# scottschroeder/shirley-raytracing-rs

Hardware: AMD Instinct MI355X
Metric: Msamples/sec (whole node) on book-1 random_scene 1200x800 @ 500spp; 1/2/4/8 GPU (higher is better)
Workload: dtype f64

## Files before the change

### include/shirley_rt.h

```cpp
#ifndef SHIRLEY_RT_H
#define SHIRLEY_RT_H

#include <stddef.h>
#include <stdint.h>

#ifdef __cplusplus
extern "C" {
#endif

#define RT_ABI_VERSION 11

typedef enum rt_status {
  RT_OK = 0,
  RT_E_INVALID = 1,
  RT_E_HIP = 2,
  RT_E_OOM = 3,
  RT_E_UNSUPPORTED = 4,
  RT_E_RCCL = 5
} rt_status;

enum { RT_GEOM_SPHERE = 0, RT_GEOM_RECT_XY = 1, RT_GEOM_RECT_YZ = 2, RT_GEOM_RECT_XZ = 3, RT_GEOM_RECT_BOX = 4,
       RT_GEOM_MOVING_SPHERE = 5 };
enum { RT_MAT_METAL = 0, RT_MAT_DIELECTRIC = 1, RT_MAT_LAMBERTIAN = 2, RT_MAT_DIFFUSE_LIGHT = 3, RT_MAT_FAIRY_LIGHT = 4,
       RT_MAT_ISOTROPIC = 5 };
// ... 67 lines not shown
  int32_t n_perlin;
  const rt_perlin_table* perlin;
  int32_t n_images;
  const rt_image* images;
} rt_scene_desc;

typedef struct rt_camera {
  int32_t image_width;
  int32_t image_height;
  double height;
  double width;
  double focal_length;
  int32_t has_lens;
  double lens_radius;
  double origin[3];
  double w[3], u[3], v[3];
  double focus_length;
  double time0, time1;
} rt_camera;

typedef struct rt_render_params {
  int32_t samples;
  int32_t max_depth;
  uint64_t seed;
  int32_t tile_rank;
  int32_t tile_world;
  int32_t sample_chunk;
  int32_t engine;
  int32_t sample_begin;
  int32_t sample_count;
  int32_t partition;
  int32_t scratch_mb;
} rt_render_params;

enum {
  RT_PARTITION_AUTO = 0,
  RT_PARTITION_TILES = 1,
  RT_PARTITION_SAMPLES = 2
};

typedef struct rt_scene_stats {
  int32_t n_objects;
  int32_t n_nodes;
  int32_t n_leaves;
  int32_t depth;
  int64_t device_bytes;
  int32_t n_nodes4;
  int32_t wide_block;
  double origin_limit;
  int32_t hop_pass;
  int32_t hop_kind;
} rt_scene_stats;

typedef struct rt_counters {
  uint64_t samples;
  uint64_t segments;
  uint64_t node_visits;
  uint64_t prim_tests;
  double kernel_ms;
  double reduce_ms;
  int32_t engine;
  int32_t iterations;
  uint64_t slots;
  double extend_ms;
  double shade_ms;
  double texture_ms;
  int32_t sample_chunk;
  int32_t n_chunks;
  int32_t passes;
  int32_t trace_launches;
  uint64_t scratch_bytes;
} rt_counters;

typedef struct rt_ctx rt_ctx;

const char* rt_version(void);
int rt_device_count(int32_t* out);
int rt_create(int32_t device, rt_ctx** out);
int rt_destroy(rt_ctx* ctx);
const char* rt_last_error(const rt_ctx* ctx);

int rt_scene_upload(rt_ctx* ctx, const rt_scene_desc* scene, int32_t bvh_builder);
int rt_scene_stats_get(rt_ctx* ctx, rt_scene_stats* out);
int rt_scene_digest(rt_ctx* ctx, uint64_t* out);
int rt_scene_digest_host(const rt_scene_desc* scene, int32_t bvh_builder, uint64_t* out);

int rt_render(rt_ctx* ctx, const rt_camera* cam, const rt_render_params* params, double* accum_host);

int rt_render_scanlines(rt_ctx* ctx, const rt_camera* cam, const rt_render_params* params,
                        int32_t line_begin, int32_t line_end, double* rows_host);

int rt_tile_layout(const rt_camera* cam, int32_t tile_world, int32_t* n_tiles_total, int32_t* max_tiles_per_rank);
int rt_render_device(rt_ctx* ctx, const rt_camera* cam, const rt_render_params* params, double* accum_dev,
                     void* stream);
int rt_render_tiles_device(rt_ctx* ctx, const rt_camera* cam, const rt_render_params* params,
                           double* packed_dev, void* stream);
int rt_unpack_tiles_device(rt_ctx* ctx, const rt_camera* cam, int32_t tile_world, const double* gathered_dev,
                           double* accum_dev, void* stream);
int rt_synchronize(rt_ctx* ctx);

typedef struct rt_hit {
  int32_t object;
  int32_t front_face;
  double t;
  double point[3];
  double normal[3];
  double u, v;
} rt_hit;
int rt_scene_hit(rt_ctx* ctx, const double* rays, int32_t n, double t_min, double t_max, rt_hit* out);

enum { RT_TRAVERSAL_BINARY = 0, RT_TRAVERSAL_RENDER = 1 };
int rt_scene_hit_ex(rt_ctx* ctx, const double* rays, int32_t n, double t_min, double t_max, int32_t traversal,
                    rt_hit* out);

typedef struct rt_probe {
  int32_t object;
  int32_t front_face;
  int32_t scattered;
  int32_t emits;
  uint32_t draw;
  int32_t pad;
  double t, point[3], normal[3];
  double emitted[3];
  double attenuation[3];
  double origin[3], direction[3];
} rt_probe;
int rt_probe_segment(rt_ctx* ctx, const double* rays, int32_t n, uint64_t seed, uint32_t sample, uint32_t draw,
                     rt_probe* out);

#define RT_COMM_ID_BYTES 128
typedef struct rt_comm rt_comm;
int rt_comm_unique_id(uint8_t id[RT_COMM_ID_BYTES]);
int rt_comm_init_rank(rt_ctx* ctx, const uint8_t id[RT_COMM_ID_BYTES], int32_t world, int32_t rank, rt_comm** out);
int rt_comm_destroy(rt_comm* comm);
int rt_render_sharded(rt_ctx* ctx, rt_comm* comm, const rt_camera* cam, const rt_render_params* params,
                      double* accum_dev, void* stream);
int rt_render_multi(rt_ctx* const* ctxs, int32_t n, const rt_camera* cam, const rt_render_params* params,
                    double* accum_host);

int rt_counters_get(rt_ctx* ctx, rt_counters* out);

typedef struct rt_bvh_node {
  double box[6];
  int32_t leaf;
  int32_t lhs, rhs;
  int32_t pad;
} rt_bvh_node;
int rt_bvh_build_host(const rt_scene_desc* scene, int32_t bvh_builder, int32_t* n_nodes, rt_bvh_node* nodes,
                      int32_t* root);

int rt_tonemap(const double* accum, int32_t width, int32_t height, int32_t samples, uint8_t* rgb8);
int rt_tonemap_device(rt_ctx* ctx, const double* accum_dev, int32_t width, int32_t height, int32_t samples,
                      uint8_t* rgb8_dev, void* stream);

typedef struct rt_adaptive_params {
  int32_t min_samples;
  int32_t step;
  double  threshold;
  double  noise_floor;
} rt_adaptive_params;

typedef struct rt_adaptive_report {
  int32_t  steps, tiles, tiles_converged, pad;
  uint64_t samples, segments;
  double   kernel_ms, fold_ms;
} rt_adaptive_report;
// ... 93 lines not shown
```

### shirley-raytracing-rs_amd/csrc/rt/rt_api.cpp

```cpp
#include <algorithm>
#include <cmath>
#include <cstdlib>
#include <cstring>
#include <limits>
#include <string>
#include <vector>

#include "adaptive.h"
#include "plan.h"
#include "rt_ctx.h"

using namespace rt;

namespace rt {

int ensure(rt_ctx* c, DevBuf& b, size_t bytes) {
  if (b.bytes >= bytes && b.p) return RT_OK;
  if (c) HIP_TRY(c, hipSetDevice(c->device));
  if (b.p) {
    (void)hipFree(b.p);
    b.p = nullptr;
    b.bytes = 0;
  }
  if (bytes == 0) return RT_OK;
// ... 288 lines not shown
  kp.work.tiles_x = L.tiles_x;
  kp.work.tiles_y = L.tiles_y;
  kp.work.ty0 = ty0;
  kp.work.tile_rank = p->tile_rank;
  kp.work.tile_world = p->tile_world;
  kp.work.n_tiles_rank = L.n_tiles_rank;
  kp.work.chunk = chunk;
  kp.work.max_depth = p->max_depth;
  kp.work.seed = p->seed;
  kp.work.div_tiles_x = make_udiv((uint32_t)L.tiles_x);
  kp.work.tile_list = step ? step->list_dev : nullptr;
  kp.partial = static_cast<double*>(c->partial.p);
  kp.counters = static_cast<DCounters*>(c->counters.p);

  st = ensure(c, c->kcam, (size_t)passes * sizeof(KBlock));
  if (st) return st;
  kp.scene.shutter = &static_cast<KBlock*>(c->kcam.p)->scene.time0;
  c->host_blocks.assign(passes, KBlock{});
  const uint64_t nseg = (uint64_t)std::max(1, c->cu_count * std::max(1, c->blocks_per_cu));
  {
    const size_t bytes = std::max<size_t>(64, (size_t)nseg * sizeof(uint32_t));
    st = ensure(c, c->unit_counter, bytes);
    if (st) return st;
    kp.unit_counter = static_cast<unsigned long long*>(c->unit_counter.p);
  }
  if ((int)c->pass_ev.size() < 2 * passes) {
    const size_t have = c->pass_ev.size();
    c->pass_ev.resize(2 * passes, nullptr);
    for (size_t i = have; i < c->pass_ev.size(); ++i) HIP_TRY(c, hipEventCreate(&c->pass_ev[i]));
  }
  HIP_TRY(c, hipMemsetAsync(c->counters.p, 0, kCounterSlots * sizeof(DCounters), s));
  c->last_engine = engine;
  c->host_samples = 0;
  c->last_chunk = chunk;
  c->last_n_chunks = n_chunks;
  c->last_passes = 0;
  c->last_scratch = partial_bytes;
  c->last_iters = 0;
  c->last_slots = 0;
  c->last_timing = 0;
  for (double& x : c->lap_ms) x = 0.0;
  HIP_TRY(c, hipEventRecord(c->ev[0], s));
  const bool trace = n_pix > 0 && count > 0 && p->max_depth > 0;
  if (step && (!trace || chunk != step->batch)) return fail(c, RT_E_INVALID, "bad adaptive step");
  if (!trace) {
    uint64_t inside = 0;
    for (long long lt = 0; lt < L.n_tiles_rank; ++lt) {
      const long long gt = lt * p->tile_world + p->tile_rank;
      const int tx = (int)(gt % L.tiles_x), ty = ty0 + (int)(gt / L.tiles_x);
      const int w = std::min(kTile, cam->image_width - tx * kTile), h = std::min(kTile, cam->image_height - ty * kTile);
      if (w > 0 && h > 0) inside += (uint64_t)w * (uint64_t)h;
    }
    c->host_samples = inside * (uint64_t)count;
    HIP_TRY(c, hipEventRecord(c->ev[1], s));
    if (n_pix > 0)
      HIP_TRY(c, launch_reduce(kp.partial, 0, L.n_tiles_rank, L.tiles_x, ty0, p->tile_rank, p->tile_world,
                               cam->image_width, row0, row1, packed, 0, out_dev, s));
    HIP_TRY(c, hipEventRecord(c->ev[2], s));
    c->have_timing = true;
    return RT_OK;
  }
  for (int k = 0; k < passes; ++k) {
    const int c0 = k * per_pass, c1 = std::min(n_chunks, c0 + per_pass);
    DWork& w = kp.work;
    w.sample_base = R.begin + c0 * chunk;
    w.samples = (int)std::min<long long>(R.end, (long long)R.begin + (long long)c1 * chunk);
    w.n_chunks = c1 - c0;
    w.n_units = (uint64_t)n_pix * (uint64_t)w.n_chunks;
    w.div_unit_tile = make_udiv((uint32_t)w.n_chunks * (uint32_t)kTilePixels);
    const uint64_t per = (w.n_units + nseg - 1) / nseg;
    w.n_segs = plan.segments ? (uint32_t)nseg : 0u;
    w.seg_len = (uint32_t)std::max<uint64_t>(kSegmentWindow, (per + kSegmentWindow - 1) / kSegmentWindow * kSegmentWindow);
    w.q_window = plan.queue_window;
    if (const char* e = getenv("SHIRLEY_WINDOW"))
      w.q_window = (uint32_t)std::max(1, atoi(e) / kWave) * (uint32_t)kWave;
    KBlock& kb = c->host_blocks[k];
    kb.cam = kp.cam;
    kb.scene = kp.scene;
    kb.work = w;
    kb.partial = kp.partial;
    kb.unit_counter = kp.unit_counter;
    kb.counters = kp.counters;
    kb.ground = c->place.hop_kind == 2 ? static_cast<const DGround*>(c->ground.p) : nullptr;
    void* kdev = static_cast<KBlock*>(c->kcam.p) + k;
    HIP_TRY(c, hipMemcpyAsync(kdev, &kb, sizeof(KBlock), hipMemcpyHostToDevice, s));
    kp.kconst = (uint64_t)(uintptr_t)kdev;
    HIP_TRY(c, hipMemsetAsync(c->unit_counter.p, 0, std::max<size_t>(64, (size_t)nseg * sizeof(uint32_t)), s));
    HIP_TRY(c, hipEventRecord(c->pass_ev[2 * k], s));
    if (engine == RT_ENGINE_WAVEFRONT) {
      st = run_wavefront(c, kp, timing, s);
      if (st) return st;
    } else if (engine == RT_ENGINE_SPLIT) {
      kp.split_refill = c->split_refill;
      KParams ks = kp;
      ks.scene.n_lds_mats = ks.scene.n_lds_texs = 0;
      HIP_TRY(c, launch_split(ks, c->split_nt, c->cu_count, s));
    } else {
      HIP_TRY(c, launch_trace(kp, (int)nseg, c->place.mk_threads, hop_instance(c->place), s));
    }
    HIP_TRY(c, hipEventRecord(c->pass_ev[2 * k + 1], s));
    if (k == passes - 1) HIP_TRY(c, hipEventRecord(c->ev[1], s));
    if (step)
      HIP_TRY(c, launch_fold_stats(kp.partial, w.n_chunks, step->n_list, step->list_dev, L.tiles_x, cam->image_width,
                                   cam->image_height, step->batches_before + c1, step->batch, step->noise_floor,
                                   out_dev, step->moments_dev, step->err_dev, s));
    else
      HIP_TRY(c, launch_reduce(kp.partial, w.n_chunks, L.n_tiles_rank, L.tiles_x, ty0, p->tile_rank, p->tile_world,
                               cam->image_width, row0, row1, packed, k > 0 ? 1 : 0, out_dev, s));
    c->last_passes = k + 1;
  }
  HIP_TRY(c, hipEventRecord(c->ev[2], s));
  c->have_timing = true;
  return RT_OK;
}

}

extern "C" {

const char* rt_version(void) { return "shirley-rt 0.2 (gfx950, f64 wavefront + persistent megakernel)"; }

int rt_device_count(int32_t* out) {
  if (!out) return RT_E_INVALID;
  int n = 0;
  hipError_t e = hipGetDeviceCount(&n);
  *out = (e == hipSuccess) ? n : 0;
  return e == hipSuccess ? RT_OK : RT_E_HIP;
}

const char* rt_last_error(const rt_ctx* ctx) { return ctx ? ctx->err.c_str() : "NULL context"; }

int rt_create(int32_t device, rt_ctx** out) {
  if (!out) return RT_E_INVALID;
  *out = nullptr;
  int n = 0;
  if (hipGetDeviceCount(&n) != hipSuccess || n == 0) return RT_E_HIP;
  if (device < 0 || device >= n) return RT_E_INVALID;
  rt_ctx* c = new rt_ctx();
  c->device = device;
  auto bail = [&](int code) {
    rt_destroy(c);
    return code;
  };
  if (hipSetDevice(device) != hipSuccess) return bail(RT_E_HIP);
  if (hipStreamCreateWithFlags(&c->stream, hipStreamNonBlocking) != hipSuccess) return bail(RT_E_HIP);
  hipDeviceProp_t prop;
  if (hipGetDeviceProperties(&prop, device) != hipSuccess) return bail(RT_E_HIP);
  c->cu_count = prop.multiProcessorCount;
  for (auto& e : c->ev)
    if (hipEventCreate(&e) != hipSuccess) return bail(RT_E_HIP);
  for (auto& e : c->wf_ev)
    if (hipEventCreate(&e) != hipSuccess) return bail(RT_E_HIP);
  if (hipHostMalloc((void**)&c->wf_host, 64, hipHostMallocDefault) != hipSuccess) return bail(RT_E_OOM);
  if (ensure(c, c->counters, kCounterSlots * sizeof(DCounters)) || ensure(c, c->unit_counter, 64)) return bail(RT_E_OOM);
  *out = c;
  return RT_OK;
}

int rt_destroy(rt_ctx* c) {
  if (!c) return RT_OK;
  (void)hipSetDevice(c->device);
  if (c->stream) (void)hipStreamSynchronize(c->stream);
  for (DevBuf* b : {&c->nodes, &c->nodes4, &c->prims, &c->mats, &c->texs, &c->perlin, &c->texels, &c->exts, &c->ground, &c->lights, &c->prim_light, &c->light_cdf, &c->partial, &c->kcam, &c->shutter0, &c->moments, &c->tile_list, &c->tile_err, &c->dn_a, &c->dn_b, &c->feat,
                    &c->accum, &c->counters, &c->unit_counter, &c->wf_pool, &c->wf_iters, &c->packed, &c->gathered,
                    &c->parts, &c->band, &c->digests})
    release(*b);
  for (rt_comm& m : c->group_comms)
    if (m.comm) (void)rccl().CommDestroy(m.comm);
  for (auto& e : c->ev)
    if (e) (void)hipEventDestroy(e);
  for (auto& e : c->wf_ev)
    if (e) (void)hipEventDestroy(e);
  for (auto& e : c->lap_ev) (void)hipEventDestroy(e);
  if (c->wf_host) (void)hipHostFree(c->wf_host);
  if (c->stream) (void)hipStreamDestroy(c->stream);
  delete c;
  return RT_OK;
}

int rt_scene_upload(rt_ctx* c, const rt_scene_desc* d, int32_t builder) {
  if (!c) return RT_E_INVALID;
  CompiledScene cs;
  int st = compile_scene(d, builder, tuning_from_env(), &cs, &c->err);
  if (st) return st;
  const ScenePlacement& P = cs.place;
  HIP_TRY(c, hipSetDevice(c->device));
  HIP_TRY(c, hipStreamSynchronize(c->stream));
  c->have_scene = false;
  auto up = [&](DevBuf& b, const auto& v) { return upload(c, b, v.data(), v.size() * sizeof v[0]); };
  if ((st = up(c->nodes, cs.nodes)) || (st = up(c->nodes4, cs.nodes4)) || (st = up(c->prims, cs.prims)) ||
      (st = up(c->mats, cs.mats)) || (st = up(c->texels, cs.texels)))
    return st;
  for (DTex& t : cs.texs)
    if (t.kind == RT_TEX_IMAGE) t.img.texels = static_cast<const uint8_t*>(c->texels.p) + cs.img_off[t.table];
  if ((st = up(c->texs, cs.texs)) || (st = up(c->perlin, cs.perlin))) return st;
  if (!cs.exts.empty()) {
    if ((st = up(c->exts, cs.exts))) return st;
  } else {
    release(c->exts);
  }
  if (!cs.ground.empty()) {
    if ((st = up(c->ground, cs.ground))) return st;
  } else {
    release(c->ground);
  }
  if (!cs.lights.dev.empty()) {
    if ((st = up(c->lights, cs.lights.dev))) return st;
  } else {
    release(c->lights);
  }
  if ((st = up(c->prim_light, cs.prim_light))) return st;
  if ((st = ensure(c, c->shutter0, 2 * sizeof(double)))) return st;
  HIP_TRY(c, hipMemset(c->shutter0.p, 0, 2 * sizeof(double)));

  DScene& S = c->scene;
  S.nodes = static_cast<const DNode*>(c->nodes.p);
  S.nodes4 = c->nodes4.p;
  S.prims = static_cast<const DPrim*>(c->prims.p);
  S.mats = static_cast<const DMat*>(c->mats.p);
  S.texs = static_cast<const DTex*>(c->texs.p);
  S.perlin = static_cast<const DPerlin*>(c->perlin.p);
  S.exts = cs.exts.empty() ? nullptr : static_cast<const DExt*>(c->exts.p);
  S.time0 = S.time1 = 0.0;
  S.shutter = static_cast<const double*>(c->shutter0.p);
  S.n_nodes = (int32_t)cs.nodes.size();
  S.n_nodes4 = cs.stats.n_nodes4;
  S.n_prims = cs.stats.n_objects;
  place_scene(P, S);
  S.sky = d->sky;
  for (int k = 0; k < 3; ++k) S.sky_color[k] = d->sky_color[k];
  c->place = P;

  int bpc = 0;
  HIP_TRY(c, trace_occupancy(S, P.mk_threads, hop_instance(P), &bpc));
  if (bpc < 1) return fail(c, RT_E_UNSUPPORTED, "trace kernel does not fit on a CU (LDS %lld B)", P.stack_bytes);
  c->blocks_per_cu = bpc;
  DScene W = S;
  W.n_lds_mats = W.n_lds_texs = 0;
  W.n_lds_nodes = P.wf_n_lds_nodes;
  int wbpc = 0;
  HIP_TRY(c, wf_prepare(W, &wbpc));
  if (wbpc < 1) return fail(c, RT_E_UNSUPPORTED, "wavefront extend kernel does not fit on a CU");
  c->wf_scene = W;
  c->wf_blocks_per_cu = wbpc;
  c->wf_wide = false;
  if (P.wf_extend4) {
    int b4 = 0;
    HIP_TRY(c, wf_prepare4(S, &b4));
    if (b4 >= 1) {
      c->wf_wide = true;
      c->wf4_blocks_per_cu = b4;
      c->wf_scene = S;
      c->wf_scene.n_lds_mats = c->wf_scene.n_lds_texs = 0;
    }
  }
  c->split_nt = 0;
  if (P.split_nt) {
    if (P.split_refill) c->split_refill = P.split_refill;
    int sb = 0;
    if (split_supported_nt(P.split_nt)) HIP_TRY(c, split_prepare(S, P.split_nt, &sb));
    if (sb >= 1) c->split_nt = P.split_nt;
  }

  c->n_perlin = cs.n_perlin;
  c->has_perlin = cs.has_perlin;
  c->prim_object = std::move(cs.prim_object);
  c->uv_fixups = std::move(cs.uv_fixups);
  c->light_list = std::move(cs.lights.lights);
  c->light_dev = std::move(cs.lights.dev);
  c->light_cells = 0;
  c->n_unlisted_lights = cs.lights.n_unlisted;
  c->stats = cs.stats;
  c->digest = cs.digest;
  c->have_scene = true;
  return RT_OK;
}
int rt_scene_digest(rt_ctx* c, uint64_t* out) {
  if (!c || !out) return RT_E_INVALID;
  if (!c->have_scene) return fail(c, RT_E_INVALID, "no scene uploaded");
  *out = c->digest;
  return RT_OK;
}

int rt_scene_digest_host(const rt_scene_desc* d, int32_t builder, uint64_t* out) {
  if (!d || !out) return RT_E_INVALID;
  if (validate(d, nullptr)) return RT_E_INVALID;
  *out = scene_digest(d, builder & ~kPlacementMask);
  return RT_OK;
}

int rt_scene_stats_get(rt_ctx* c, rt_scene_stats* out) {
  if (!c || !out) return RT_E_INVALID;
  if (!c->have_scene) return fail(c, RT_E_INVALID, "no scene uploaded");
  *out = c->stats;
  return RT_OK;
}

int rt_tile_layout(const rt_camera* cam, int32_t world, int32_t* n_tiles_total, int32_t* max_tiles_per_rank) {
  if (!cam || world < 1 || cam->image_width < 1 || cam->image_height < 1) return RT_E_INVALID;
  int tiles_y = (cam->image_height + kTile - 1) / kTile;
  Layout L = layout(cam, 0, tiles_y, 0, world);
  if (n_tiles_total) *n_tiles_total = L.n_tiles;
  if (max_tiles_per_rank) *max_tiles_per_rank = (L.n_tiles + world - 1) / world;
  return RT_OK;
}

int rt_render_device(rt_ctx* c, const rt_camera* cam, const rt_render_params* p, double* accum_dev, void* stream) {
  if (!accum_dev) return fail(c, RT_E_INVALID, "accum_dev is NULL");
  hipStream_t s;
  resolve_stream(c, stream, &s);
  int tiles_y = cam ? (cam->image_height + kTile - 1) / kTile : 0;
  SampleRange R;
  if (p && resolve_range(c, p, &R)) return RT_E_INVALID;
  return render_window(c, cam, p, R, 0, tiles_y, 0, cam ? cam->image_height : 0, 0, accum_dev, s);
}

int rt_render_tiles_device(rt_ctx* c, const rt_camera* cam, const rt_render_params* p, double* packed_dev,
                           void* stream) {
  if (!packed_dev) return fail(c, RT_E_INVALID, "packed_dev is NULL");
  hipStream_t s;
  resolve_stream(c, stream, &s);
  int tiles_y = cam ? (cam->image_height + kTile - 1) / kTile : 0;
  SampleRange R;
  if (p && resolve_range(c, p, &R)) return RT_E_INVALID;
  return render_window(c, cam, p, R, 0, tiles_y, 0, cam ? cam->image_height : 0, 1, packed_dev, s);
}

int rt_unpack_tiles_device(rt_ctx* c, const rt_camera* cam, int32_t world, const double* gathered_dev,
                           double* accum_dev, void* stream) {
  if (!c || !cam || !gathered_dev || !accum_dev || world < 1) return fail(c, RT_E_INVALID, "bad unpack args");
  hipStream_t s;
  resolve_stream(c, stream, &s);
  int32_t n_total = 0, max_tiles = 0;
  rt_tile_layout(cam, world, &n_total, &max_tiles);
  int tiles_x = (cam->image_width + kTile - 1) / kTile;
  HIP_TRY(c, hipSetDevice(c->device));
  HIP_TRY(c, launch_unpack(gathered_dev, world, max_tiles, n_total, tiles_x, cam->image_width, cam->image_height,
                           accum_dev, s));
  return RT_OK;
}

int rt_render(rt_ctx* c, const rt_camera* cam, const rt_render_params* p, double* accum_host) {
  if (!c) return RT_E_INVALID;
  if (!accum_host || !cam) return fail(c, RT_E_INVALID, "NULL argument");
  return rt_render_scanlines(c, cam, p, 0, cam->image_height, accum_host);
}

int rt_render_scanlines(rt_ctx* c, const rt_camera* cam, const rt_render_params* p, int32_t line_begin,
                        int32_t line_end, double* rows_host) {
  if (!c) return RT_E_INVALID;
  if (!cam || !rows_host) return fail(c, RT_E_INVALID, "NULL argument");
  if (line_begin < 0 || line_end > cam->image_height || line_begin > line_end)
    return fail(c, RT_E_INVALID, "bad line range [%d, %d)", line_begin, line_end);
  if (line_begin == line_end) return RT_OK;
  if (p && p->tile_world != 1) return fail(c, RT_E_INVALID, "host-buffer render needs tile_world == 1");
  size_t bytes = (size_t)(line_end - line_begin) * cam->image_width * 3 * sizeof(double);
  int st = ensure(c, c->accum, bytes);
  if (st) return st;
  int ty0 = line_begin / kTile, ty1 = (line_end + kTile - 1) / kTile;
  SampleRange R;
  if (p && resolve_range(c, p, &R)) return RT_E_INVALID;
  st = render_window(c, cam, p, R, ty0, ty1, line_begin, line_end, 0, static_cast<double*>(c->accum.p), c->stream);
  if (st) return st;
  HIP_TRY(c, hipMemcpyAsync(rows_host, c->accum.p, bytes, hipMemcpyDeviceToHost, c->stream));
  HIP_TRY(c, hipStreamSynchronize(c->stream));
  return RT_OK;
}

int rt_scene_hit(rt_ctx* c, const double* rays, int32_t n, double t_min, double t_max, rt_hit* out) {
  return rt_scene_hit_ex(c, rays, n, t_min, t_max, RT_TRAVERSAL_BINARY, out);
}

int rt_scene_hit_ex(rt_ctx* c, const double* rays, int32_t n, double t_min, double t_max, int32_t traversal,
                    rt_hit* out) {
  if (!c) return RT_E_INVALID;
  if (!c->have_scene) return fail(c, RT_E_INVALID, "no scene uploaded");
  if (n < 0 || (n > 0 && (!rays || !out))) return fail(c, RT_E_INVALID, "bad ray batch");
  if (traversal != RT_TRAVERSAL_BINARY && traversal != RT_TRAVERSAL_RENDER)
    return fail(c, RT_E_INVALID, "bad traversal %d", traversal);
  if (n == 0) return RT_OK;
  static_assert(sizeof(rt_hit) == 80, "rt_hit layout");
  HIP_TRY(c, hipSetDevice(c->device));
  DevBuf r, h;
  int st = upload(c, r, rays, (size_t)n * 6 * sizeof(double));
  if (!st) st = ensure(c, h, (size_t)n * sizeof(rt_hit));
  if (!st) {
    const double* rd = static_cast<const double*>(r.p);
    hipError_t e = traversal == RT_TRAVERSAL_RENDER
                       ? launch_hit4(c->scene, c->place.wide, rd, n, t_min, t_max, h.p, c->stream)
                       : launch_hit(c->scene, rd, n, t_min, t_max, h.p, c->stream);
    if (e == hipSuccess) e = hipMemcpyAsync(out, h.p, (size_t)n * sizeof(rt_hit), hipMemcpyDeviceToHost, c->stream);
    if (e == hipSuccess) e = hipStreamSynchronize(c->stream);
    if (e != hipSuccess) st = fail(c, RT_E_HIP, "rt_scene_hit: %s", hipGetErrorString(e));
  }
  if (!st)
    for (int32_t i = 0; i < n; ++i)
      if (out[i].object >= 0) out[i].object = c->prim_object[out[i].object];
  if (!st && !c->uv_fixups.empty())
    for (int32_t i = 0; i < n; ++i) {
      auto it = std::lower_bound(c->uv_fixups.begin(), c->uv_fixups.end(), out[i].object,
                                 [](const auto& f, int32_t o) { return f.first < o; });
      if (it != c->uv_fixups.end() && it->first == out[i].object) instance_sphere_uv(it->second.first, it->second.second, out[i]);
    }
  release(r);
  release(h);
  return st;
}

int rt_probe_segment(rt_ctx* c, const double* rays, int32_t n, uint64_t seed, uint32_t sample, uint32_t draw,
                     rt_probe* out) {
  if (!c) return RT_E_INVALID;
  if (!c->have_scene) return fail(c, RT_E_INVALID, "no scene uploaded");
  if (n < 0 || (n > 0 && (!rays || !out))) return fail(c, RT_E_INVALID, "bad ray batch");
  if (n == 0) return RT_OK;
  static_assert(sizeof(rt_probe) == 176, "rt_probe layout (trace.hip ProbeOut)");
  HIP_TRY(c, hipSetDevice(c->device));
  DevBuf r, h;
  int st = upload(c, r, rays, (size_t)n * 6 * sizeof(double));
  if (!st) st = ensure(c, h, (size_t)n * sizeof(rt_probe));
  if (!st) {
    DScene S = c->scene;
    S.time0 = S.time1 = 0.0;
    hipError_t e = launch_probe(S, c->place.wide, static_cast<const double*>(r.p), n, seed,
                                sample, draw, h.p, c->stream);
    if (e == hipSuccess) e = hipMemcpyAsync(out, h.p, (size_t)n * sizeof(rt_probe), hipMemcpyDeviceToHost, c->stream);
    if (e == hipSuccess) e = hipStreamSynchronize(c->stream);
    if (e != hipSuccess) st = fail(c, RT_E_HIP, "rt_probe_segment: %s", hipGetErrorString(e));
  }
  if (!st)
    for (int32_t i = 0; i < n; ++i)
      if (out[i].object >= 0) out[i].object = c->prim_object[out[i].object];
  release(r);
  release(h);
  return st;
}

int rt_synchronize(rt_ctx* c) {
  if (!c) return RT_E_INVALID;
  HIP_TRY(c, hipSetDevice(c->device));
  HIP_TRY(c, hipDeviceSynchronize());
  return RT_OK;
}

int rt_counters_get(rt_ctx* c, rt_counters* out) {
  if (!c || !out) return RT_E_INVALID;
  std::memset(out, 0, sizeof *out);
  if (!c->have_timing) return fail(c, RT_E_INVALID, "no render has run on this context");
  HIP_TRY(c, hipSetDevice(c->device));
  HIP_TRY(c, hipEventSynchronize(c->ev[2]));
  std::vector<DCounters> dc(kCounterSlots);
  HIP_TRY(c, hipMemcpy(dc.data(), c->counters.p, kCounterSlots * sizeof(DCounters), hipMemcpyDeviceToHost));
  out->samples = c->host_samples;
  for (const DCounters& k : dc) {
    out->samples += k.samples;
    out->segments += k.segments;
    out->node_visits += k.node_visits;
    out->prim_tests += k.prim_tests;
  }
#ifdef RT_PHASE_TIMING
  {
    double ph[kPhBuckets] = {};
    for (const DCounters& k : dc)
      for (int i = 0; i < kPhBuckets; ++i) ph[i] += (double)k.pad[i];
    const int order[] = {kPhTrav, kPhRecord, kPhRegen, kPhMarble, kPhDraws, kPhCamera, kPhShade, kPhTail};
    const char* names[] = {"trav", "record", "regen", "marble", "draws", "camera", "shade", "tail"};
    double tot = 0;
    for (int b : order) tot += ph[b];
    fprintf(stderr, "[phase] wave-time fractions:");
    for (int i = 0; i < 8; ++i) fprintf(stderr, " %s %.4f", names[i], ph[order[i]] / tot);
    fprintf(stderr, " (wave-cycles %.4g)\n", tot);
    const double lane = ph[kPhLaneSteps], wave = ph[kPhWaveSteps];
    fprintf(stderr, "[phase] traversal lane steps %.4g, wave steps %.4g, SIMD utilisation %.3f\n", lane, wave,
            lane / (64.0 * wave));
    phase_counters_dump();
  }
#endif
#ifdef RT_TIMELINE
  timeline_dump();
#endif
  float all = 0.f;
  HIP_TRY(c, hipEventElapsedTime(&all, c->ev[0], c->ev[2]));
  double trace = 0.0;
  for (int k = 0; k < c->last_passes; ++k) {
    float t = 0.f;
    HIP_TRY(c, hipEventElapsedTime(&t, c->pass_ev[2 * k], c->pass_ev[2 * k + 1]));
    trace += t;
  }
  out->kernel_ms = trace;
  out->reduce_ms = std::max(0.0, (double)all - trace);
  out->passes = c->last_passes;
  out->trace_launches = c->last_passes;
  out->scratch_bytes = c->last_scratch;
  out->engine = c->last_engine;
  out->sample_chunk = c->last_chunk;
  out->n_chunks = c->last_n_chunks;
  out->iterations = c->last_iters;
  out->slots = c->last_slots;
  if (c->last_timing) {
    out->extend_ms = c->lap_ms[0];
    out->shade_ms = c->lap_ms[1];
    out->texture_ms = c->lap_ms[2];
  }
  return RT_OK;
}

int rt_bvh_build_host(const rt_scene_desc* d, int32_t builder, int32_t* n_nodes, rt_bvh_node* nodes, int32_t* root) {
  if (!d || !n_nodes) return RT_E_INVALID;
  if (validate(d, nullptr)) return RT_E_INVALID;
  std::vector<rt_object> flat;
  const rt_scene_desc fd = flat_scene(d, flat);
  BuiltTree t = build_tree(&fd, builder, tuning_from_env());
  if (nodes) {
    if (*n_nodes < (int32_t)t.nodes.size()) return RT_E_INVALID;
    for (size_t i = 0; i < t.nodes.size(); ++i) {
      box_to6(t.nodes[i].box, nodes[i].box);
      nodes[i].leaf = t.nodes[i].leaf;
      nodes[i].lhs = t.nodes[i].lhs;
      nodes[i].rhs = t.nodes[i].rhs;
      nodes[i].pad = 0;
    }
  }
  *n_nodes = (int32_t)t.nodes.size();
  if (root) *root = t.root;
  return RT_OK;
}

int rt_tonemap(const double* accum, int32_t width, int32_t height, int32_t samples, uint8_t* rgb8) {
  if (!accum || !rgb8 || width < 1 || height < 1) return RT_E_INVALID;
  const double inv = 1.0 / (double)(samples == 0 ? 1 : samples);
  for (int32_t j = 0; j < height; ++j)
    for (int32_t i = 0; i < width; ++i) {
      const double* c = accum + ((size_t)j * width + i) * 3;
      uint8_t* o = rgb8 + ((size_t)(height - j - 1) * width + i) * 3;
      for (int k = 0; k < 3; ++k) {
        double y = std::sqrt(c[k] * inv) * 255.999;
        o[k] = (std::isnan(y) || y <= 0.0) ? 0 : (y >= 255.0 ? 255 : (uint8_t)y);
      }
    }
  return RT_OK;
}

int rt_tonemap_device(rt_ctx* c, const double* accum_dev, int32_t width, int32_t height, int32_t samples,
                      uint8_t* rgb8_dev, void* stream) {
  if (!c || !accum_dev || !rgb8_dev || width < 1 || height < 1) return RT_E_INVALID;
  hipStream_t s;
  resolve_stream(c, stream, &s);
  HIP_TRY(c, hipSetDevice(c->device));
  const double inv = 1.0 / (double)(samples == 0 ? 1 : samples);
  HIP_TRY(c, launch_tonemap(accum_dev, width, height, inv, rgb8_dev, s));
  return RT_OK;
}

// ... 123 lines not shown
```

### shirley-raytracing-rs_amd/csrc/rt/rt_ctx.h

```cpp
#pragma once

#include <hip/hip_runtime.h>

#include <cstdarg>
#include <cstdio>
#include <string>
#include <utility>
#include <vector>

#include "../../../include/shirley_rt.h"
#include "keycheck.h"
#include "light_pick.h"
#include "rccl_loader.h"
#include "rt_launch.h"
#include "rt_layout.h"
#include "scene_compile.h"

struct DevBuf {
  void* p = nullptr;
  size_t bytes = 0;
};

struct rt_comm {
  ncclComm_t comm = nullptr;
  int world = 1, rank = 0, device = 0;
  rt::KeyState ks;
  uint64_t* key_words = nullptr;
  hipEvent_t key_ev[2] = {nullptr, nullptr};
  int key_slot = 0;
  int key_pending = 0;
};

struct rt_ctx {
  int device = 0;
  hipStream_t stream = nullptr;
  std::string err;
  int cu_count = 0;
  bool have_scene = false;
  rt::DScene scene{};
  DevBuf nodes, nodes4, prims, mats, texs, perlin, texels, exts;
  DevBuf ground;
  DevBuf lights;
  DevBuf prim_light;
  std::vector<rt_light> light_list;
  std::vector<rt::DLight> light_dev;
  int32_t light_cells = 0;
  DevBuf light_cdf;
  rt::DLightGrid light_grid{};
  rt_light_grid light_grid_info{};
  int32_t n_unlisted_lights = 0;
  rt_scene_stats stats{};
  int blocks_per_cu = 0;
  rt::ScenePlacement place;
  int split_nt = 0;
  int split_refill = 8;
  rt::DScene wf_scene{};
  int wf_blocks_per_cu = 0;
  bool wf_wide = false;
  int wf4_blocks_per_cu = 0;
  bool has_perlin = false;
  int n_perlin = 0;
  DevBuf partial, accum, counters, unit_counter, kcam;
  DevBuf moments, tile_list, tile_err;
  DevBuf dn_a, dn_b;
  DevBuf feat;
  DevBuf shutter0;
  DevBuf wf_pool, wf_iters;
  uint32_t* wf_host = nullptr;
  hipEvent_t ev[3] = {nullptr, nullptr, nullptr};
  hipEvent_t wf_ev[2] = {nullptr, nullptr};
  std::vector<hipEvent_t> lap_ev;
  bool have_timing = false;
  int last_engine = 0, last_iters = 0, last_timing = 0, last_chunk = 0, last_n_chunks = 0, last_passes = 0;
  uint64_t last_slots = 0, last_scratch = 0;
  std::vector<hipEvent_t> pass_ev;
  std::vector<rt::KBlock> host_blocks;
  uint64_t digest = 0;
  std::vector<int32_t> prim_object;
  std::vector<std::pair<int32_t, std::pair<double, double>>> uv_fixups;
  uint64_t host_samples = 0;
  double lap_ms[3] = {0, 0, 0};
  DevBuf packed, gathered, parts, band, digests;
  std::vector<int> group_devices;
  std::vector<rt_comm> group_comms;
};

namespace rt {

inline int fail(rt_ctx* c, int code, const char* fmt, ...) {
  char buf[512];
  va_list ap;
  va_start(ap, fmt);
  vsnprintf(buf, sizeof buf, fmt, ap);
  va_end(ap);
  if (c) c->err = buf;
  return code;
}

#define HIP_TRY(ctx, expr)                                                                      \
  do {                                                                                          \
    hipError_t e_ = (expr);                                                                     \
    if (e_ != hipSuccess)                                                                       \
      return fail(ctx, e_ == hipErrorOutOfMemory ? RT_E_OOM : RT_E_HIP, "%s: %s (%s:%d)", #expr, \
                  hipGetErrorString(e_), __FILE__, __LINE__);                                   \
  } while (0)

DCamera device_camera(const rt_camera* c);
int ensure(rt_ctx* c, DevBuf& b, size_t bytes);
void release(DevBuf& b);
int upload(rt_ctx* c, DevBuf& b, const void* src, size_t bytes);

inline int resolve_stream(rt_ctx* c, void* stream, hipStream_t* out) {
  *out = stream ? reinterpret_cast<hipStream_t>(stream) : c->stream;
  return RT_OK;
}

struct Layout {
  int tiles_x, tiles_y, n_tiles, n_tiles_rank;
};

inline Layout layout(const rt_camera* cam, int ty0, int ty1, int rank, int world) {
  Layout L;
  L.tiles_x = (cam->image_width + kTile - 1) / kTile;
  L.tiles_y = ty1 - ty0;
// ... 84 lines not shown
```

### shirley-raytracing-rs_amd/csrc/rt/rt_device.h

```cpp
#pragma once

#ifdef RT_PORTABLE_LIBM
#include "portable_libm.h"
#define RT_SIN pl_sin
#define RT_LOG pl_log
#define RT_ACOS pl_acos
#define RT_ATAN2 pl_atan2
#define RT_POW5_LIBM(x) pl_pow5(x)
#else
#define RT_SIN sin
#define RT_LOG log
#define RT_ACOS acos
#define RT_ATAN2 atan2
#define RT_POW5_LIBM(x) pow(x, 5.0)
#endif
#include <hip/hip_runtime.h>

#include "../../../include/shirley_rt.h"
#include "rt_layout.h"

namespace rt {


struct v3 {
// ... 752 lines not shown
    if (next < 0) {
      resolve_ties<EXT>(S, o, d, t_min, T.t_best, T.best, T.face, rk, seed);
      return true;
    }
  }
  T.node = next;
  return false;
}

template <int STRIDE, int MODE, bool EXT>
__device__ __forceinline__ int traverse(const DScene& S, const DNode* lds_nodes, v3 o, v3 d, double t_min,
                                        double& t_best, int& face_best, const Rng& rk, uint64_t seed,
                                        int* stk_node, float* stk_t, unsigned& visits, unsigned& ptests) {
  const v3 inv = V(1.0 / d.x, 1.0 / d.y, 1.0 / d.z);
  const RaySigns ns = ray_signs(inv);
  const double a = len2(d);
  int best = -1;
  int sp = 0;
  int node = 0;
  for (int steps = 0; steps < S.n_nodes; ++steps) {
    const DNode& nd = fetch_node<MODE>(S, lds_nodes, node);
    const int c0 = nd.child[0], c1 = nd.child[1];
    double te0 = 0.0, te1 = 0.0;
    bool h0 = (c0 != kEmptyChild) && slab_s(nd.box[0], o, inv, ns, t_min, t_best, te0);
    bool h1 = (c1 != kEmptyChild) && slab_s(nd.box[1], o, inv, ns, t_min, t_best, te1);
    visits += (c0 != kEmptyChild ? 1u : 0u) + (c1 != kEmptyChild ? 1u : 0u);
    mark_tie<EXT>(best, (!h0 && near_entry(te0, t_best)) || (!h1 && near_entry(te1, t_best)));
    if (h0 && c0 < 0) {
      const DPrim& pr = S.prims[~c0];
      double t;
      int f = -1;
      ++ptests;
      if (prim_t<EXT>(S, pr, ~c0, o, d, a, t_min, t_best, rk, seed, t, f) &&
          tie_takes<EXT>(S, ~c0, best, t, t_best, o, inv, ns, t_min)) {
        t_best = t;
        best = ~c0;
        face_best = f;
      }
      h0 = false;
    }
    if (h1 && c1 < 0) {
      const DPrim& pr = S.prims[~c1];
      double t;
      int f = -1;
      ++ptests;
      if (prim_t<EXT>(S, pr, ~c1, o, d, a, t_min, t_best, rk, seed, t, f) &&
          tie_takes<EXT>(S, ~c1, best, t, t_best, o, inv, ns, t_min)) {
        t_best = t;
        best = ~c1;
        face_best = f;
      }
      h1 = false;
    }
    int next;
    if (h0 && h1) {
      const bool first0 = te0 <= te1;
      next = first0 ? c0 : c1;
      stk_node[sp * STRIDE] = first0 ? c1 : c0;
      stk_t[sp * STRIDE] = __double2float_rd(first0 ? te1 : te0);
      ++sp;
    } else if (h0) {
      next = c0;
    } else if (h1) {
      next = c1;
    } else {
      next = -1;
      while (sp > 0) {
        --sp;
        if ((double)stk_t[sp * STRIDE] <= t_best) {
          next = stk_node[sp * STRIDE];
          break;
        }
      }
      if (next < 0) break;
    }
    node = next;
  }
  resolve_ties<EXT>(S, o, d, t_min, t_best, best, face_best, rk, seed);
  return best;
}

#ifdef RT_PHASE_TIMING
#define g_trav_lane_steps trav_lane_steps_ref
constexpr int kPhaseEvents = 48;
static __device__ unsigned long long g_phase_ctr[2 * kPhaseEvents];
static __device__ unsigned long long g_visit_hist[64], g_wave_visit_hist[64];

__device__ __forceinline__ void ph_count(int i) {
  const unsigned long long act = __ballot(1);
  if ((int)__lane_id() == __builtin_ctzll(act)) {
    atomicAdd(&g_phase_ctr[2 * i], (unsigned long long)__popcll(act));
    atomicAdd(&g_phase_ctr[2 * i + 1], 1ull);
  }
}
#ifndef RT_PHASE_NO_EVENTS
#define PH_COUNT(i) ph_count(i)
#else
#define PH_COUNT(i)
#endif
#else
#define PH_COUNT(i)
#endif
#ifdef RT_PHASE_TIMING
#define RT_STAT(x) x
#define RT_STAT_ARG(x) , x
#else
#define RT_STAT(x)
#define RT_STAT_ARG(x)
#endif
#ifdef RT_TIMELINE
constexpr int kTimelineWaves = 1 << 16;
static __device__ unsigned long long g_wave_t0[kTimelineWaves], g_wave_tx[kTimelineWaves], g_wave_t1[kTimelineWaves];
#endif
template <int MODE, class N4>
__device__ __forceinline__ const N4& fetch_node4(const DScene& S, const N4* lds_nodes, int idx) {
  if (MODE == kNodesLds || MODE == kSceneLds)
    return *reinterpret_cast<const N4*>(reinterpret_cast<const char*>(lds_nodes) +
                                        __umul24((unsigned)idx, (unsigned)sizeof(N4)));
  const N4* g = static_cast<const N4*>(S.nodes4);
  if (MODE == kNodesGlobal) return g[idx];
  return (idx < S.n_lds_nodes4) ? lds_nodes[idx] : g[idx];
}

struct RayF {
  float ox, oy, oz, ix, iy, iz, oix, oiy, oiz;
  bool fast;
  int dx, dy, dz;
};
template <class N4>
__device__ __forceinline__ RayF ray_f(const DScene& S, v3 o, v3 inv) {
  RayF r;
  r.ox = (float)o.x;
  r.oy = (float)o.y;
  r.oz = (float)o.z;
  r.ix = (float)inv.x;
  r.iy = (float)inv.y;
  r.iz = (float)inv.z;
  r.oix = r.ox * r.ix;
  r.oiy = r.oy * r.iy;
  r.oiz = r.oz * r.iz;
  r.fast = fmax(fmax(fabs(o.x), fabs(o.y)), fabs(o.z)) <= (double)S.origin_limit;
  r.dx = r.ix < 0.f ? N4::kNegRow : 0;
  r.dy = r.iy < 0.f ? N4::kNegRow : 0;
  r.dz = r.iz < 0.f ? N4::kNegRow : 0;
  return r;
}

typedef float f32x2 __attribute__((ext_vector_type(2)));
__device__ __forceinline__ f32x2 f2(float a, float b) { return f32x2{a, b}; }
__device__ __forceinline__ f32x2 pk_fma(f32x2 a, f32x2 b, f32x2 c) { return __builtin_elementwise_fma(a, b, c); }

template <bool M1, class N4>
__device__ __forceinline__ void node4_keys(const N4& nd, const RayF& r, v3 o, v3 inv, float tminf, float tmaxf,
                                           double t_min, double t_max, float& k0, float& k1, float& k2, float& k3,
                                           const int4& ch, unsigned (&hc)[4]) {
  const unsigned chw[4] = {(unsigned)ch.x, (unsigned)ch.y, (unsigned)ch.z, (unsigned)ch.w};
  const char* nb = reinterpret_cast<const char*>(&nd);
  float4 nx4, fx4, ny4, fy4, nz4, fz4;
  if constexpr (N4::kRows3) {
    const char* bx = nb + r.dx;
    const char* by = nb + r.dy;
    const char* bz = nb + r.dz;
    nx4 = *reinterpret_cast<const float4*>(bx);
    fx4 = *reinterpret_cast<const float4*>(bx + 16);
    ny4 = *reinterpret_cast<const float4*>(by + 48);
    fy4 = *reinterpret_cast<const float4*>(by + 64);
    nz4 = *reinterpret_cast<const float4*>(bz + 96);
    fz4 = *reinterpret_cast<const float4*>(bz + 112);
  } else {
// ... 351 lines not shown
  S.root4 = __builtin_amdgcn_readfirstlane(root4);
  S.key_mask = (unsigned)__builtin_amdgcn_readfirstlane((int)key_mask);
  S.origin_limit = __int_as_float(__builtin_amdgcn_readfirstlane(__float_as_int(origin_limit)));
  RootHit r{0, -1, -1, __builtin_inf()};
  unsigned visits = 0, ptests = 0;
  r.ok = traverse4_root<MODE>(S, lds_nodes, lds_prims, o, d, 0.001, r.t, r.best, r.face, rk, uniform64(seed_v), visits,
                              ptests)
             ? 1
             : 0;
  return r;
}
#endif

__device__ __forceinline__ bool box_inward(int face, v3 d) {
  const double da = face < 2 ? d.z : (face < 4 ? d.x : d.y);
  return (face & 1) ? da > 0.0 : da < 0.0;
}
typedef __attribute__((address_space(4))) const DGround GGround;
constexpr int kHopRefused = 0, kHopServed = 1, kHopFound = 2;
template <bool DOWN>
__device__ __forceinline__ int ground_hop_t(const DScene& S, const DPrim* lds_prims, const DMat* mats, GGround* g, v3 o, v3 d,
                                            double t_min, double& t_best, int& best, int& face_best, bool& guarded) {
  bool div_ok;
  const v3 inv = inv_dir(d, div_ok);
  const RaySigns ns = ray_signs(inv);
  t_best = __builtin_inf();
  best = -1;
  face_best = -1;
  const int n = g->n, n_box = g->n_box;
#pragma unroll 1
  for (int i = 0; i < n; ++i) {
    const int leaf = g->prim[i];
    const DPrim& pr = lds_prims[leaf];
    double te, t;
    if (i < n_box) {
      double tx;
      if (!slab_s(pr.p, o, inv, ns, t_min, t_best, te, tx)) {
        mark_tie<false>(best, near_entry(te, t_best));
        continue;
      }
      const int f = div_ok ? box_t1f(pr.p, o, d, inv, ns, t_min, t_best, te, tx, t) : box_t(pr.p, o, d, t_min, t_best, t, inv, div_ok);
      if (f >= 0 && tie_takes<false>(S, leaf, best, t, t_best, o, inv, ns, t_min)) { t_best = t; best = leaf; face_best = f; }
    } else {
      double b[6];
      leaf_box(pr, b);
      if (!slab_s(b, o, inv, ns, t_min, t_best, te)) continue;
      if (rect_t<0, 2>(pr.p, o, d, t_min, t_best, t, inv, div_ok) && tie_takes<false>(S, leaf, best, t, t_best, o, inv, ns, t_min)) {
        t_best = t; best = leaf; face_best = -1;
      }
    }
  }
  guarded = false;
  if (best < 0 || (best & kTieBit) || (DOWN ? face_best >= 0 && face_best < 4 : face_best < 4) || !(t_best > t_min))
    return kHopRefused;
  const DPrim& pb = lds_prims[best];
  const double ay = fabs(d.y);
  const bool diel = mats[pb.material].kind == RT_MAT_DIELECTRIC;
  const bool slab_ok = o.y >= g->y_lo && o.y <= g->y_hi && ay >= g->dy_min && ay <= 0x1p300 &&
                       d.x * d.x + d.z * d.z <= g->ratio2 * (d.y * d.y);
  if constexpr (DOWN) {
    if (!diel) {
      const double y = face_best < 0 ? pb.p[4] + 0.0001 : (face_best == 4 ? pb.p[4] : pb.p[1]);
      return (slab_ok && y <= g->y_down) ? kHopFound : kHopRefused;
    }
    if (face_best < 4) return kHopRefused;
  }
  bool ok = diel && slab_ok;
  if (ok && (face_best == 4 ? pb.p[4] : pb.p[1]) == g->y_top) {
    const int nx = g->nx;
    const int ix = ground_cell(o.x + t_best * d.x, g->x0, nx), iz = ground_cell(o.z + t_best * d.z, g->z0, g->nz);
    if (ix >= 0 && iz >= 0) {
      typedef __attribute__((address_space(1))) const uint32_t GBits;
      const unsigned c = (unsigned)iz * (unsigned)nx + (unsigned)ix;
      GBits* bits = (GBits*)(uintptr_t)((uint64_t)(uintptr_t)g + sizeof(DGround));
      guarded = (bits[c >> 5] >> (c & 31u)) & 1u;
      ok = !guarded;
    }
  }
  return ok ? kHopServed : kHopRefused;
}
__device__ __forceinline__ bool ground_hop(const DScene& S, const DPrim* lds_prims, const DMat* mats, GGround* g, v3 o, v3 d,
                                           double t_min, double& t_best, int& best, int& face_best, bool& guarded) {
  return ground_hop_t<false>(S, lds_prims, mats, g, o, d, t_min, t_best, best, face_best, guarded) != kHopRefused;
}

struct Trav4 {
  v3 inv;
  Recip ra;
  bool ra_ok;
  double t_best;
  float tmaxf;
  int best, face, node, sp, steps;
  unsigned top;
  RaySigns ns;
  RayF rf;
};

template <bool EXT>
__device__ __forceinline__ void trav4_begin(Trav4& T, const DScene& S, v3 o, v3 d, double t_max) {
  bool inv_ok;
  T.inv = inv_dir(d, inv_ok);
  T.ns = ray_signs(T.inv);
  T.rf = ray_f<typename Node4Sel<EXT>::T>(S, o, T.inv);
  T.ra = recip(len2(d));
  T.ra_ok = inv_ok && T.ra.b >= 0x1p-300 && T.ra.b <= 0x1p300 && T.rf.fast;
  T.t_best = t_max;
  T.tmaxf = tmax_f32(t_max);
  T.best = -1;
  T.face = -1;
  T.node = S.root4;
  T.sp = 0;
  T.top = ~0u;
  T.steps = 0;
}

template <int STRIDE, int MODE, bool EXT>
__device__ __forceinline__ bool trav4_step(const DScene& S, const typename Node4Sel<EXT>::T* lds_nodes, const DPrim* lds_prims, v3 o,
                                           v3 d, double t_min, Trav4& T, unsigned* stk, const Rng& rk,
                                           uint64_t seed, unsigned& visits, unsigned& ptests) {
  if (++T.steps > S.n_nodes4) {
    T.best = strip_tie(T.best);
    return true;
  }
  unsigned xdefer = 0u;
  T.node = visit4<STRIDE, MODE, EXT>(S, lds_nodes, lds_prims, o, d, T.inv, T.ns, T.rf, T.ra, T.ra_ok, t_min, T.node, T.t_best,
                                     T.tmaxf, T.best, T.face, T.sp, T.top, stk, rk, seed, visits, ptests, xdefer);
  if (T.node >= 0) return false;
  resolve_ties<EXT>(S, o, d, t_min, T.t_best, T.best, T.face, rk, seed);
  return true;
}

template <int MODE, class N4>
__device__ __forceinline__ void stage_nodes4(const DScene& S, N4* lds_nodes, DPrim* lds_prims) {
  if (MODE == kNodesGlobal) return;
  const int4* src = reinterpret_cast<const int4*>(S.nodes4);
  int4* dst = reinterpret_cast<int4*>(lds_nodes);
  const int n16 = S.n_lds_nodes4 * (int)(sizeof(N4) / 16);
  for (int i = threadIdx.x; i < n16; i += blockDim.x) dst[i] = src[i];
  if (MODE == kSceneLds) {
    const int4* ps = reinterpret_cast<const int4*>(S.prims);
    int4* pd = reinterpret_cast<int4*>(lds_prims);
    const int p16 = S.n_lds_prims * (int)(sizeof(DPrim) / 16);
    for (int i = threadIdx.x; i < p16; i += blockDim.x) pd[i] = ps[i];
    const int4* ts = reinterpret_cast<const int4*>(S.perlin);
    int4* td = reinterpret_cast<int4*>(lds_prims + S.n_lds_prims);
    const int t16 = S.n_lds_perlin * (int)(sizeof(DPerlin) / 16);
    for (int i = threadIdx.x; i < t16; i += blockDim.x) td[i] = ts[i];
    if (S.n_lds_mats > 0) {
      const int4* ms = reinterpret_cast<const int4*>(S.mats);
      int4* md = td + t16;
      const int m16 = S.n_lds_mats * (int)(sizeof(DMat) / 16);
      for (int i = threadIdx.x; i < m16; i += blockDim.x) md[i] = ms[i];
      const int4* xs = reinterpret_cast<const int4*>(S.texs);
      int4* xd = md + m16;
      const int x16 = S.n_lds_texs * (int)(sizeof(DTex) / 16);
      for (int i = threadIdx.x; i < x16; i += blockDim.x) xd[i] = xs[i];
    }
  }
  __syncthreads();
}

template <int MODE>
__device__ __forceinline__ void stage_nodes(const DScene& S, DNode* lds_nodes) {
  if (MODE == kNodesGlobal) return;
  const int4* src = reinterpret_cast<const int4*>(S.nodes);
  int4* dst = reinterpret_cast<int4*>(lds_nodes);
// ... 707 lines not shown
```

### shirley-raytracing-rs_amd/csrc/rt/rt_layout.h

```cpp
#pragma once

#include <stddef.h>
#include <stdint.h>

#include "plan.h"

namespace rt {

constexpr int kTile = 8;
constexpr int kTilePixels = kTile * kTile;
constexpr int kTraceThreads = 256;
constexpr int kTraceThreadsWide = 1024;
#ifndef RT_EXT_WIDE_THREADS
#define RT_EXT_WIDE_THREADS 768
#endif
constexpr int kTraceThreadsWide3 = RT_EXT_WIDE_THREADS;
constexpr int kHitThreads = 256;
constexpr int kExtendThreads = 256;
constexpr int kWave = 64;
constexpr int kLdsBytes = 160 * 1024;

constexpr int32_t kEmptyChild = 0x7fffffff;
struct alignas(16) DNode {
  double box[2][6];
// ... 67 lines not shown
  const uint8_t* texels;
  int32_t width, height;
};
struct alignas(16) DTex {
  int32_t kind;
  int32_t odd, even, table;
  union {
    double color[3];
    DTexImage img;
  };
  double scale;
};
static_assert(sizeof(DTex) == 48, "DTex layout");

struct DPerlin {
  double ranfloat[256][3];
  int32_t perm_x[256], perm_y[256], perm_z[256];
};

inline constexpr size_t trace_lds_bytes(int n_lds_nodes4, int node4_size, int n_lds_prims, int n_lds_perlin,
                                        int stack_depth4, int threads, int n_lds_mats, int n_lds_texs) {
  return (size_t)n_lds_nodes4 * node4_size + (size_t)n_lds_prims * sizeof(DPrim) +
         (size_t)n_lds_perlin * sizeof(DPerlin) + (size_t)n_lds_mats * sizeof(DMat) + (size_t)n_lds_texs * sizeof(DTex) +
         (size_t)stack_depth4 * threads * kStack4EntryBytes;
}
inline size_t wf_extend_lds(int n_lds_nodes, int stack_depth) {
  return (size_t)n_lds_nodes * sizeof(DNode) + (size_t)stack_depth * kExtendThreads * 8;
}

struct DScene {
  const DNode* nodes;
  const DPrim* prims;
  const DMat* mats;
  const DTex* texs;
  const DPerlin* perlin;
  int32_t n_nodes, n_prims;
  int32_t stack_depth;
  int32_t n_lds_nodes;
  const void* nodes4;
  int32_t n_nodes4;
  int32_t stack_depth4;
  int32_t n_lds_nodes4;
  int32_t n_lds_prims;
  int32_t n_lds_perlin;
  float origin_limit;
  int32_t root4;
  uint32_t key_mask;
  int32_t sky;
  double sky_color[3];
  const DExt* exts;
  double time0, time1;
  const double* shutter;
  int32_t n_lds_mats;
  int32_t n_lds_texs;
};

constexpr int kGroundMaxPrims = 4;
constexpr double kGroundCellsPerUnit = 32.0;
constexpr double kGroundCell = 1.0 / kGroundCellsPerUnit;
constexpr double kGroundGuard = 1.0 / 32.0;
constexpr long long kGroundMaxCells = 128LL * 1024 * 8;
struct alignas(16) DGround {
  double y_lo, y_hi;
  double y_top;
  double dy_min;
  double ratio2;
  double x0, z0;
  int32_t nx, nz;
  int32_t n, n_box;
  int32_t prim[kGroundMaxPrims];
  double y_down;
};
static_assert(sizeof(DGround) == 96, "DGround layout");
#ifdef __HIPCC__
#define RT_HOST_DEVICE __host__ __device__
#else
#define RT_HOST_DEVICE
#endif
RT_HOST_DEVICE inline int ground_cell(double v, double v0, int n) {
  const double q = (v - v0) * kGroundCellsPerUnit;
  return (q >= 0.0 && q < (double)n) ? (int)q : -1;
}

struct DCamera {
  int32_t width, height;
  int32_t has_lens;
  int32_t pad;
  double lens_radius;
  double origin[3], u[3], v[3];
  double horizontal[3], vertical[3], lower_left[3];
  double wd, hd, inv_w, inv_h;
};

struct UDiv {
  uint32_t m, s1, s2;
};
inline UDiv make_udiv(uint32_t d) {
  uint32_t l = 0;
  while (l < 32 && (1ull << l) < d) ++l;
  const uint64_t m = (((1ull << l) - d) << 32) / d + 1;
  return UDiv{(uint32_t)m, l < 1 ? l : 1u, l > 0 ? l - 1 : 0u};
}

struct DWork {
  UDiv div_unit_tile;
  UDiv div_tiles_x;
  int32_t tiles_x, tiles_y;
  int32_t tile_rank, tile_world;
  int32_t n_tiles_rank;
  int32_t samples;
  int32_t sample_base;
  int32_t chunk;
  int32_t n_chunks;
  int32_t max_depth;
  int32_t ty0;
  uint64_t seed;
  uint64_t n_units;
  uint32_t seg_len, n_segs;
  uint32_t q_window, pad_q;
  const uint32_t* tile_list;
};

struct DCounters {
  unsigned long long samples, segments, node_visits, prim_tests;
  unsigned long long pad[12];
};
constexpr int kCounterSlots = 64;
enum : int {
  kPhRegen = 0, kPhTrav = 1, kPhShade = 2, kPhLaneSteps = 3, kPhWaveSteps = 4, kPhRecord = 5, kPhMarble = 6,
  kPhDraws = 7, kPhCamera = 8, kPhTail = 9, kPhBuckets = 10
};

struct KParams {
  DScene scene;
  DCamera cam;
  DWork work;
  double* partial;
  unsigned long long* unit_counter;
  DCounters* counters;
  int32_t split_refill;
  uint64_t kconst;
};

struct alignas(16) KBlock {
  DCamera cam;
  DScene scene;
  DWork work;
  double* partial;
  unsigned long long* unit_counter;
  DCounters* counters;
  const DGround* ground;
};

struct WfState {
  double *ox, *oy, *oz, *dx, *dy, *dz;
  double *ax, *ay, *az;
  double *ex, *ey, *ez;
  double *sx, *sy, *sz;
  double* ht;
  uint64_t* part;
  uint32_t* pixel;
  uint32_t *sample, *draw, *c2, *c3;
  int32_t *s_next, *s_end;
  int32_t* depth;
  int32_t *hprim, *hface;
  uint8_t* state;
};
constexpr size_t kWfSlotBytes = 16 * 8 + 8 + 11 * 4 + 1;

struct WfTexQ {
  double *px, *py, *pz, *scale;
  int32_t *slot, *tex, *kind;
  uint32_t* count;
};
constexpr size_t kWfTexBytes = 4 * 8 + 3 * 4;

constexpr int kWfQueues = 64;
struct WfIter {
  unsigned long long fetch[kWfQueues][16];
};

struct WfParams {
  DScene scene;
  DCamera cam;
  DWork work;
  WfState st;
  WfTexQ tq;
  uint32_t n_slots;
  uint32_t first;
  int32_t n_perlin;
  uint32_t ext_window;
  double* partial;
  unsigned long long* unit_counter;
  unsigned long long* win;
  unsigned* retired;
  DCounters* counters;
  WfIter* it;
};

struct alignas(16) DLight {
  int32_t geometry;
  int32_t emitter;
  int32_t pad[2];
  double p[6];
  double area;
  double color[3];
};
static_assert(sizeof(DLight) == 96, "DLight layout");

}
```

### shirley-raytracing-rs_amd/csrc/rt/scene_compile.cpp

```cpp
#include "scene_compile.h"

#include <algorithm>
#include <cmath>
#include <cstdarg>
#include <cstdio>
#include <cstdlib>
#include <cstring>
#include <limits>

namespace rt {

namespace {
int fail(std::string* err, int code, const char* fmt, ...) {
  char buf[512];
  va_list ap;
  va_start(ap, fmt);
  vsnprintf(buf, sizeof buf, fmt, ap);
  va_end(ap);
  if (err) *err = buf;
  return code;
}
}

SceneTuning tuning_from_env() {
  SceneTuning t;
  if (const char* e = getenv("SHIRLEY_COLLAPSE_DP")) t.collapse_dp = atoi(e) != 0;
  if (const char* e = getenv("SHIRLEY_LDS_NODES")) {
    t.has_lds_nodes = true;
    t.lds_nodes = atoll(e);
  }
  t.no_wide = getenv("SHIRLEY_NO_WIDE") != nullptr;
  t.no_lds_prims = getenv("SHIRLEY_NO_LDS_PRIMS") != nullptr;
  t.no_lds_mats = getenv("SHIRLEY_NO_LDS_MATS") != nullptr;
  t.no_lds_perlin = getenv("SHIRLEY_NO_LDS_PERLIN") != nullptr;
  t.no_hop = getenv("SHIRLEY_NO_HOP") != nullptr;
  if (const char* e = getenv("SHIRLEY_HOP")) {
    t.hop_root = std::strcmp(e, "root") == 0;
    t.hop_up = std::strcmp(e, "up") == 0;
  }
  if (const char* e = getenv("SHIRLEY_SAH_BOXW")) t.sah_box_weight = atof(e);
  t.sah_binned = getenv("SHIRLEY_SAH_BINNED") != nullptr;
  t.wf_extend2 = getenv("SHIRLEY_WF_EXTEND2") != nullptr;
  if (const char* e = getenv("SHIRLEY_SPLIT_NT")) t.split_nt = atoi(e);
  if (const char* e = getenv("SHIRLEY_SPLIT_REFILL")) t.split_refill = std::max(1, atoi(e));
  return t;
}

bool is_extended(const rt_object& o) {
  return o.geometry == RT_GEOM_MOVING_SPHERE || o.medium != 0 || o.transform != 0;
}
void rotate_y_cs(const rt_object& o, double& cs, double& sn) {
  const double rad = o.rotate_y_deg * 3.14159265358979323846 / 180.0;
  cs = std::cos(rad);
  sn = std::sin(rad);
}
bool texture_uses_uv(const rt_scene_desc* d, int32_t ti) {
  if (ti < 0 || ti >= d->n_textures) return false;
  const rt_texture& t = d->textures[ti];
  if (t.kind == RT_TEX_IMAGE) return true;
  if (t.kind == RT_TEX_CHECKER) return texture_uses_uv(d, t.odd) || texture_uses_uv(d, t.even);
  return false;
}
bool flattens(const rt_scene_desc* d, const rt_object& o) {
  if (o.geometry != RT_GEOM_SPHERE || !o.transform || o.medium) return false;
  if (o.rotate_y_deg == 0.0) return true;
  return o.material >= 0 && o.material < d->n_materials && !texture_uses_uv(d, d->materials[o.material].texture);
}
rt_object flat_object(const rt_scene_desc* d, const rt_object& o) {
  rt_object f = o;
  if (!flattens(d, o)) return f;
  double cs, sn;
  rotate_y_cs(o, cs, sn);
  const double cx = o.p[0], cy = o.p[1], cz = o.p[2];
  f.p[0] = (cs * cx + sn * cz) + o.offset[0];
  f.p[1] = cy + o.offset[1];
  f.p[2] = (-sn * cx + cs * cz) + o.offset[2];
  f.transform = 0;
  f.rotate_y_deg = 0.0;
  f.offset[0] = f.offset[1] = f.offset[2] = 0.0;
  return f;
}
rt_scene_desc flat_scene(const rt_scene_desc* d, std::vector<rt_object>& store) {
  store.resize((size_t)std::max(0, d->n_objects));
  for (int i = 0; i < d->n_objects; ++i) store[i] = flat_object(d, d->objects[i]);
  rt_scene_desc f = *d;
  f.objects = store.data();
  return f;
}
void instance_sphere_uv(double cs, double sn, rt_hit& h) {
  const double s = h.front_face ? 1.0 : -1.0;
  const double nx = s * h.normal[0], ny = s * h.normal[1], nz = s * h.normal[2];
  const double ox = cs * nx - sn * nz, oz = sn * nx + cs * nz;
  const double pi = 3.14159265358979323846;
  h.u = (std::atan2(-oz, ox) + pi) / (2.0 * pi);
  h.v = std::acos(-ny) / pi;
}
void moving_center(const rt_object& o, double tm, double* c) {
  const double s = (tm - o.q[3]) / (o.q[4] - o.q[3]);
  for (int k = 0; k < 3; ++k) c[k] = o.p[k] + (o.q[k] - o.p[k]) * s;
}

Box reference_box(const rt_object& o);
Box object_box(const rt_object& o) {
  if (!is_extended(o)) return reference_box(o);
  Box b{};
  if (o.geometry == RT_GEOM_MOVING_SPHERE) {
    double c0[3], c1[3];
    moving_center(o, o.q[3], c0);
    moving_center(o, o.q[4], c1);
    Box b0{}, b1{};
    for (int k = 0; k < 3; ++k) {
      b0.mn[k] = c0[k] - o.p[3];
      b0.mx[k] = c0[k] + o.p[3];
      b1.mn[k] = c1[k] - o.p[3];
      b1.mx[k] = c1[k] + o.p[3];
    }
    b = surrounding(b0, b1);
  } else {
    b = reference_box(o);
  }
  if (o.transform) {
// ... 313 lines not shown
    collect(t->nodes[n].rhs, 4 - split[n * 5 + 4], out);
  }
  void collect(int32_t c, int j, std::vector<int32_t>& out) const {
    const BuildNode& b = t->nodes[c];
    if (b.leaf >= 0 || j == 1 || !(G[c * 5 + j] < H[c * 5 + 1])) {
      out.push_back(c);
      return;
    }
    collect(b.lhs, split[c * 5 + j], out);
    collect(b.rhs, j - split[c * 5 + j], out);
  }
};

void flatten4(const BuiltTree& t, const rt_scene_desc* d, double delta, std::vector<DNode4F>& out,
              int32_t& stack_bound, bool use_dp) {
  Collapse4 dp;
  if (t.root >= 0 && use_dp) dp.build(t);
  out.clear();
  DNode4F top{};
  for (int k = 0; k < 4; ++k) {
    top.child[k] = kEmptyChild;
    set_child_box(top, k, nullptr, delta);
  }
  out.push_back(top);
  stack_bound = 1;
  if (t.root < 0) return;
  auto internal = [&](int32_t n) { return t.nodes[n].leaf < 0; };
  struct Item {
    int32_t built;
    int32_t parent;
    int slot;
    int32_t level;
  };
  std::vector<Item> q{{t.root, 0, 0, 0}};
  for (size_t head = 0; head < q.size(); ++head) {
    const Item it = q[head];
    const BuildNode& bn = t.nodes[it.built];
    set_child_box(out[it.parent], it.slot, &bn.box, delta);
    if (bn.leaf >= 0) {
      const int32_t g = d->objects[bn.leaf].geometry;
      const int32_t flags = is_extended(d->objects[bn.leaf]) ? kLeafGeneric | kLeafBox
                            : g == RT_GEOM_SPHERE            ? 0
                            : (g == RT_GEOM_RECT_BOX ? kLeafGeneric | kLeafBox : kLeafGeneric);
      out[it.parent].child[it.slot] = ~(bn.leaf | flags);
      continue;
    }
    const int32_t idx = (int32_t)out.size();
    out[it.parent].child[it.slot] = idx;
    DNode4F nd{};
    for (int k = 0; k < 4; ++k) {
      nd.child[k] = kEmptyChild;
      set_child_box(nd, k, nullptr, delta);
    }
    out.push_back(nd);
    std::vector<int32_t> ch;
    if (dp.ready()) {
      dp.children(it.built, ch);
    } else {
      ch = {bn.lhs, bn.rhs};
      while (ch.size() < 4) {
        int pick = -1;
        double best = -1.0;
        for (size_t i = 0; i < ch.size(); ++i)
          if (internal(ch[i]) && half_area(t.nodes[ch[i]].box) > best) {
            best = half_area(t.nodes[ch[i]].box);
            pick = (int)i;
          }
        if (pick < 0) break;
        const int32_t x = ch[pick];
        ch[pick] = t.nodes[x].lhs;
        ch.insert(ch.begin() + pick + 1, t.nodes[x].rhs);
      }
    }
    int n_int = 0;
    for (int32_t c : ch) n_int += internal(c) ? 1 : 0;
    const int32_t level = it.level + std::max(0, n_int - 1);
    stack_bound = std::max(stack_bound, level + 1);
    for (size_t i = 0; i < ch.size(); ++i) q.push_back({ch[i], idx, (int)i, level});
  }
}
namespace {

bool sphere_never_hit(const double* p) { return p[3] <= 0.0 && p[1] - p[3] >= p[1] + p[3]; }
bool ground_stack(const std::vector<DPrim>& prims, int n_prims, std::vector<uint32_t>& out) {
  out.clear();
  std::vector<int32_t> boxes, rects;
  double top = -std::numeric_limits<double>::infinity(), low = -top;
  double ex0 = low, ex1 = top, ez0 = low, ez1 = top, r_min = low, r_max = 0.0;
  std::vector<double> planes;
  for (int i = 0; i < n_prims; ++i) {
    const DPrim& q = prims[i];
    const double* p = q.p;
    if (q.kind == kPrimBox) {
      boxes.push_back(i);
      planes.push_back(p[1]);
      planes.push_back(p[4]);
      top = std::max(top, p[4]);
      ex0 = std::min(ex0, p[0]), ex1 = std::max(ex1, p[3]), ez0 = std::min(ez0, p[2]), ez1 = std::max(ez1, p[5]);
    } else if (q.kind == kPrimRectXZ) {
      rects.push_back(i);
      planes.push_back(p[4]);
      top = std::max(top, p[4] + 0.0001);
      ex0 = std::min(ex0, p[0]), ex1 = std::max(ex1, p[1]), ez0 = std::min(ez0, p[2]), ez1 = std::max(ez1, p[3]);
    } else if (q.kind == kPrimSphere) {
      if (!std::isfinite(p[3])) return false;
      if (sphere_never_hit(p)) continue;
      if (!(p[3] > 0.0)) return false;
      r_min = std::min(r_min, p[3]);
      r_max = std::max(r_max, p[3]);
    } else {
      return false;
    }
  }
  const size_t n_g = boxes.size() + rects.size();
  if (n_g < 1 || n_g > (size_t)kGroundMaxPrims) return false;
  for (double y : planes) low = std::min(low, y);
  const double big = 0x1p20;
  if (!(std::fabs(top) <= big && std::fabs(low) <= big && ex0 >= -big && ex1 <= big && ez0 >= -big && ez1 <= big &&
        ex0 <= ex1 && ez0 <= ez1 && r_max <= 0x1p10))
    return false;
  double dist = 0.0;
  std::vector<const DPrim*> guarded;
  for (int i = 0; i < n_prims; ++i) {
    const DPrim& q = prims[i];
    if (q.kind != kPrimSphere || sphere_never_hit(q.p)) continue;
    const double* p = q.p;
    const double lo_y = p[1] - p[3];
    if (!(lo_y >= top) || !(std::fabs(p[0]) <= big && std::fabs(p[1]) <= big && std::fabs(p[2]) <= big)) return false;
    const double dx = std::max(std::fabs(p[0] - ex0), std::fabs(p[0] - ex1));
    const double dy = std::max(std::fabs(p[1] - low), std::fabs(p[1] - top));
    const double dz = std::max(std::fabs(p[2] - ez0), std::fabs(p[2] - ez1));
    dist = std::max(dist, std::sqrt(dx * dx + dy * dy + dz * dz));
    if (lo_y - top < kGroundGuard / 2) guarded.push_back(&q);
  }
  const double ratio = 0x1p10, tol = 0x1p-40 * std::max(1.0, std::max(std::fabs(top), std::fabs(low)));
  const double reach = ((top - low) + 2.0 * tol) * (ratio + 1.0);
  const double l2 = (dist + reach) * (dist + reach) + reach * reach + r_max * r_max;
  const double m = 0x1p-38 * l2;
  const double eta = std::isfinite(r_min) ? m / (2.0 * r_min) : 0.0;
  if (!(eta <= 0x1p-16 && m <= 0x1p-13)) return false;
  const double gap = 4.0 * eta + 4.0 * tol;
  for (double y : planes)
    if (y != top && !(y <= top - gap)) return false;

  DGround g;
  std::memset(&g, 0, sizeof g);
  g.y_lo = low - tol;
  g.y_hi = top + tol;
  g.y_top = top;
  g.dy_min = std::max((2.0 * eta + 4.0 * tol) / 0.001, 0x1p-100);
  g.y_down = top - gap;
  g.ratio2 = ratio * ratio;
  g.n = (int32_t)n_g;
  g.n_box = (int32_t)boxes.size();
  for (size_t i = 0; i < boxes.size(); ++i) g.prim[i] = boxes[i];
  for (size_t i = 0; i < rects.size(); ++i) g.prim[boxes.size() + i] = rects[i];
  size_t words = 0;
  if (!guarded.empty()) {
    double cx0 = guarded[0]->p[0], cx1 = cx0, cz0 = guarded[0]->p[2], cz1 = cz0;
    for (const DPrim* q : guarded) {
      cx0 = std::min(cx0, q->p[0]), cx1 = std::max(cx1, q->p[0]);
      cz0 = std::min(cz0, q->p[2]), cz1 = std::max(cz1, q->p[2]);
    }
    g.x0 = std::floor(cx0 * kGroundCellsPerUnit - 2.0) * kGroundCell;
    g.z0 = std::floor(cz0 * kGroundCellsPerUnit - 2.0) * kGroundCell;
    const double nx = std::ceil((cx1 - g.x0) * kGroundCellsPerUnit + 2.0), nz = std::ceil((cz1 - g.z0) * kGroundCellsPerUnit + 2.0);
    if (!(nx * nz <= (double)kGroundMaxCells)) return false;
    g.nx = (int32_t)nx;
    g.nz = (int32_t)nz;
    words = ((size_t)g.nx * (size_t)g.nz + 31) / 32;
  }
  out.assign(sizeof(DGround) / 4 + words, 0u);
  std::memcpy(out.data(), &g, sizeof g);
  uint32_t* bits = out.data() + sizeof(DGround) / 4;
  const double rad = kGroundGuard * (1.0 + 0x1p-20);
  for (const DPrim* q : guarded) {
    const double cx = q->p[0], cz = q->p[2];
    const int i0 = ground_cell(cx, g.x0, g.nx), k0 = ground_cell(cz, g.z0, g.nz);
    const int span = (int)std::ceil(rad * kGroundCellsPerUnit) + 1;
    for (int k = std::max(0, k0 - span); k <= std::min(g.nz - 1, k0 + span); ++k)
      for (int i = std::max(0, i0 - span); i <= std::min(g.nx - 1, i0 + span); ++i) {
        const double x_lo = g.x0 + i * kGroundCell, z_lo = g.z0 + k * kGroundCell;
        const double dx = std::max(0.0, std::max(x_lo - cx, cx - (x_lo + kGroundCell)));
        const double dz = std::max(0.0, std::max(z_lo - cz, cz - (z_lo + kGroundCell)));
        if (dx * dx + dz * dz <= rad * rad) {
          const size_t c = (size_t)k * (size_t)g.nx + (size_t)i;
          bits[c >> 5] |= 1u << (c & 31);
        }
      }
  }
  return true;
}

int plan_placement(const rt_scene_desc* d, int32_t placement, const SceneTuning& tune, const BuiltTree& tree,
                   const std::vector<DNode4F>& nodes4, int32_t stack4, float origin_limit, CompiledScene& cs,
                   std::string* err) {
  ScenePlacement& P = cs.place;
  const bool ext = !cs.exts.empty();
  const int n_nodes4 = (int)nodes4.size(), n_mats = (int)cs.mats.size(), n_texs = (int)cs.texs.size();
  P.stack_depth4 = stack4;
  P.root4 = (nodes4[0].child[0] >= 0 && nodes4[0].child[0] != kEmptyChild) ? nodes4[0].child[0] : 0;
  {
    int kbits = 1;
    while ((size_t)1 << kbits < nodes4.size()) ++kbits;
    if (kbits > kMaxKeyBits) return fail(err, RT_E_UNSUPPORTED, "BVH too large (%zu 4-wide nodes)", nodes4.size());
    P.key_mask = (1u << kbits) - 1u;
  }
  P.origin_limit = origin_limit;
  const int32_t depth = tree_branch_depth(tree);
  P.stack_depth = depth + 2;
  auto lds_count = [&](long long stack, size_t node_bytes, size_t n) -> int32_t {
    long long room = std::min<long long>((kLdsBytes - stack) / (long long)node_bytes, (long long)n);
    if (placement & RT_BVH_NODES_LDS) return (int32_t)room;
    if (placement & RT_BVH_NODES_HALF_LDS) return (int32_t)std::min<long long>(room, (long long)n / 2);
    if (tune.has_lds_nodes) return (int32_t)std::min<long long>(room, tune.lds_nodes);
    return 0;
  };
  auto lds_nodes_for = [&](long long stack) { return lds_count(stack, sizeof(DNode), cs.nodes.size()); };
  P.stack_bytes = (long long)P.stack_depth * kTraceThreads * 8;
  const long long stack4_bytes = (long long)trace_lds_bytes(0, 0, 0, 0, stack4, kTraceThreads, 0, 0);
  const int wide_threads = ext ? kTraceThreadsWide3 : kTraceThreadsWide;
  const int n4_bytes = node4_bytes(ext);
  auto wide_lds = [&](int n_prims, int n_perlin, int mats, int texs) {
    return trace_lds_bytes(n_nodes4, n4_bytes, n_prims, n_perlin, stack4, wide_threads, mats, texs);
  };
  if (P.stack_bytes > kLdsBytes || stack4_bytes > kLdsBytes)
    return fail(err, RT_E_UNSUPPORTED, "BVH too deep for the LDS traversal stack (depth %d)", depth);
  P.wide = wide_lds(0, 0, 0, 0) <= (size_t)kLdsBytes && (placement == 0 || placement == RT_BVH_NODES_LDS) &&
           !tune.no_wide;
  P.mk_threads = P.wide ? wide_threads : kTraceThreads;
  P.n_lds_nodes = lds_nodes_for(kHitThreads * 8LL * P.stack_depth);
  P.n_lds_nodes4 = P.wide ? n_nodes4 : lds_count(stack4_bytes, n4_bytes, nodes4.size());
  const bool prims_lds = P.wide && wide_lds(d->n_objects, 0, n_mats, n_texs) <= (size_t)kLdsBytes &&
                         !tune.no_lds_prims && !tune.no_lds_mats;
  P.n_lds_prims = prims_lds ? d->n_objects : 0;
  const bool perlin_lds = prims_lds && d->n_perlin > 0 &&
                          wide_lds(d->n_objects, d->n_perlin, n_mats, n_texs) <= (size_t)kLdsBytes &&
                          !tune.no_lds_perlin;
  P.n_lds_perlin = perlin_lds ? d->n_perlin : 0;
  P.n_lds_mats = prims_lds ? n_mats : 0;
  P.n_lds_texs = prims_lds ? n_texs : 0;
  bool coat = false;
  for (int i = 0; i < d->n_objects && !coat; ++i) {
    const rt_object& o = d->objects[i];
    coat = o.geometry == RT_GEOM_RECT_BOX && d->materials[o.material].kind == RT_MAT_DIELECTRIC;
  }
  P.hop_pass = coat && !ext && prims_lds && !tune.no_hop;
  P.hop_kind = !P.hop_pass ? 0 : (!tune.hop_root && ground_stack(cs.prims, d->n_objects, cs.ground)) ? 2 : 1;
  if (P.hop_kind != 2) cs.ground.clear();
  P.hop_down = false;
  if (P.hop_kind == 2 && !tune.hop_up) {
    DGround g;
    std::memcpy(&g, cs.ground.data(), sizeof g);
    for (int i = 0; i < g.n && !P.hop_down; ++i) {
      const DPrim& q = cs.prims[g.prim[i]];
      if (cs.mats[q.material].kind == RT_MAT_DIELECTRIC) continue;
      P.hop_down = i < g.n_box ? (q.p[1] <= g.y_down || q.p[4] <= g.y_down) : q.p[4] + 0.0001 <= g.y_down;
    }
  }

  const long long wf_stack = (long long)wf_extend_lds(0, P.stack_depth);
  if (wf_stack > kLdsBytes)
    return fail(err, RT_E_UNSUPPORTED, "BVH too deep for the LDS traversal stack (depth %d)", depth);
  P.wf_n_lds_nodes = lds_nodes_for(wf_stack);
  P.wf_extend4 = P.wide && P.n_lds_prims > 0 && !tune.wf_extend2;
  if (P.wide && !ext && P.n_lds_prims == d->n_objects) {
    P.split_nt = tune.split_nt;
    P.split_refill = tune.split_refill;
  }

  cs.stats.n_objects = d->n_objects;
  cs.stats.n_nodes = (int32_t)tree.nodes.size();
  int32_t leaves = 0;
  for (const auto& n : tree.nodes) leaves += n.leaf >= 0;
  cs.stats.n_leaves = leaves;
  cs.stats.depth = depth;
  cs.stats.n_nodes4 = n_nodes4;
  cs.stats.wide_block = P.wide ? 1 : 0;
  cs.stats.origin_limit = P.origin_limit;
  cs.stats.hop_pass = P.hop_pass ? 1 : 0;
  cs.stats.hop_kind = P.hop_kind;
  cs.stats.device_bytes = (int64_t)(cs.nodes.size() * sizeof(DNode) + cs.prims.size() * sizeof(DPrim) +
                                    cs.mats.size() * sizeof(DMat) + cs.texs.size() * sizeof(DTex) +
                                    cs.perlin.size() * sizeof(DPerlin) + cs.texels.size());
  return RT_OK;
}

}

LightList list_lights(const rt_scene_desc* d) {
  LightList out;
  for (int i = 0; i < d->n_objects; ++i) {
    const rt_object& o = d->objects[i];
    const rt_material& m = d->materials[o.material];
    if (m.kind != RT_MAT_DIFFUSE_LIGHT && m.kind != RT_MAT_FAIRY_LIGHT) continue;
    const rt_texture& t = d->textures[m.texture];
    const bool rect = o.geometry == RT_GEOM_RECT_XY || o.geometry == RT_GEOM_RECT_YZ || o.geometry == RT_GEOM_RECT_XZ;
    bool listed = t.kind == RT_TEX_SOLID && !o.medium && !o.transform;
    double area = 0.0;
    if (rect) {
      const double e1 = o.p[1] - o.p[0], e2 = o.p[3] - o.p[2];
      listed = listed && e1 > 0.0 && e2 > 0.0;
      area = e1 * e2;
    } else if (o.geometry == RT_GEOM_SPHERE) {
      listed = listed && o.p[3] > 0.0;
      area = (4.0 * 3.141592653589793) * (o.p[3] * o.p[3]);
    } else {
      listed = false;
    }
    if (!listed) {
      ++out.n_unlisted;
      continue;
    }
    rt_light l{};
    l.object = i;
    l.geometry = o.geometry;
    l.emitter = m.kind;
    l.area = area;
    DLight dl{};
    dl.geometry = o.geometry;
    dl.emitter = m.kind;
    for (int k = 0; k < 6; ++k) dl.p[k] = o.p[k];
    dl.area = area;
    for (int k = 0; k < 3; ++k) l.color[k] = dl.color[k] = t.color[k];
    out.lights.push_back(l);
    out.dev.push_back(dl);
  }
  return out;
}

int build_light_grid(const LightList& l, int32_t cells, bool want_cdf, LightGridTable* out) {
  *out = LightGridTable{};
  if (cells < 1 || cells > kLightGridMaxCells) return RT_E_INVALID;
  const size_t L = l.dev.size();
  if (L == 0) return RT_OK;
  struct Item {
    double lo[3], hi[3], c[3], rho2, phi;
  };
  std::vector<Item> items(L);
  rt_light_grid& g = out->info;
  for (size_t j = 0; j < L; ++j) {
    const DLight& q = l.dev[j];
// ... 283 lines not shown
```

### shirley-raytracing-rs_amd/csrc/rt/scene_compile.h

```cpp
#pragma once

#include <stdint.h>

#include <string>
#include <utility>
#include <vector>

#include "../../../include/shirley_rt.h"
#include "bvh_build.h"
#include "rt_layout.h"

namespace rt {

constexpr int32_t kPlacementMask = RT_BVH_NODES_GLOBAL | RT_BVH_NODES_HALF_LDS | RT_BVH_NODES_LDS;

struct SceneTuning {
  int collapse_dp = -1;
  bool has_lds_nodes = false;
  long long lds_nodes = 0;
  bool no_wide = false;
  bool no_lds_prims = false;
  bool no_lds_mats = false;
  bool no_lds_perlin = false;
  bool no_hop = false;
  bool hop_root = false;
  bool hop_up = false;
  double sah_box_weight = 4.0;
  bool sah_binned = false;
  bool wf_extend2 = false;
  int split_nt = 8;
  int split_refill = 0;
};
SceneTuning tuning_from_env();

struct ScenePlacement {
  bool wide = false;
  int mk_threads = kTraceThreads;
  bool collapse_dp = false;
  int32_t n_lds_nodes = 0, n_lds_nodes4 = 0, n_lds_prims = 0, n_lds_perlin = 0, n_lds_mats = 0, n_lds_texs = 0;
  int32_t stack_depth = 0, stack_depth4 = 0, root4 = 0;
  long long stack_bytes = 0;
  uint32_t key_mask = 0;
  float origin_limit = 0.f;
  int32_t wf_n_lds_nodes = 0;
  bool wf_extend4 = false;
  int split_nt = 0;
  int split_refill = 0;
  bool hop_pass = false;
  int hop_kind = 0;
  bool hop_down = false;
};

inline int hop_instance(const ScenePlacement& P) { return P.hop_kind == 2 && P.hop_down ? 3 : P.hop_kind; }

inline void place_scene(const ScenePlacement& P, DScene& S) {
  S.stack_depth = P.stack_depth;
  S.stack_depth4 = P.stack_depth4;
  S.root4 = P.root4;
  S.key_mask = P.key_mask;
  S.origin_limit = P.origin_limit;
  S.n_lds_nodes = P.n_lds_nodes;
  S.n_lds_nodes4 = P.n_lds_nodes4;
  S.n_lds_prims = P.n_lds_prims;
  S.n_lds_perlin = P.n_lds_perlin;
  S.n_lds_mats = P.n_lds_mats;
  S.n_lds_texs = P.n_lds_texs;
}

struct LightList {
  std::vector<rt_light> lights;
  std::vector<DLight> dev;
  int32_t n_unlisted = 0;
};
LightList list_lights(const rt_scene_desc* d);

constexpr double kLightPickWeighted = 0.875;
constexpr double kLightPickUniform = 0.125;
constexpr int32_t kLightGridMaxCells = 64;
constexpr int64_t kLightGridMaxEntries = (int64_t)1 << 22;
struct LightGridTable {
  rt_light_grid info{};
  std::vector<double> cdf;
};
int build_light_grid(const LightList& l, int32_t cells, bool want_cdf, LightGridTable* out);

struct CompiledScene {
  std::vector<DNode> nodes;
  std::vector<unsigned char> nodes4;
  std::vector<DPrim> prims;
  std::vector<DExt> exts;
  std::vector<DMat> mats;
  std::vector<DTex> texs;
  std::vector<DPerlin> perlin;
  std::vector<uint8_t> texels;
  std::vector<size_t> img_off;
  std::vector<uint32_t> ground;
  std::vector<int32_t> prim_object;
  std::vector<std::pair<int32_t, std::pair<double, double>>> uv_fixups;
  LightList lights;
  std::vector<int32_t> prim_light;
  rt_scene_stats stats{};
  uint64_t digest = 0;
  int32_t n_perlin = 0;
  bool has_perlin = false;
  ScenePlacement place;
};

int compile_scene(const rt_scene_desc* d, int32_t builder, const SceneTuning& tune, CompiledScene* out, std::string* err);

int validate(const rt_scene_desc* d, std::string* err);

struct Fnv1a {
  uint64_t h = 14695981039346656037ull;
  void bytes(const void* p, size_t n) {
    const unsigned char* b = static_cast<const unsigned char*>(p);
    for (size_t i = 0; i < n; ++i) h = (h ^ b[i]) * 1099511628211ull;
  }
  template <class T>
  void val(const T& v) { bytes(&v, sizeof v); }
};
uint64_t scene_digest(const rt_scene_desc* d, int32_t builder);

rt_scene_desc flat_scene(const rt_scene_desc* d, std::vector<rt_object>& store);
BuiltTree build_tree(const rt_scene_desc* d, int32_t builder, const SceneTuning& tune);
void box_to6(const Box& b, double* o);
void instance_sphere_uv(double cs, double sn, rt_hit& h);

}
```

### shirley-raytracing-rs_amd/csrc/rt/trace.hip

```cpp
#include "adaptive.h"
#include "rt_device.h"
#include "pass_frame.h"
#include "rt_launch.h"

#include <algorithm>
#include <vector>

namespace rt {

__device__ __forceinline__ unsigned long long lanemask_lt() {
  unsigned lane = __lane_id();
  return (lane == 0) ? 0ull : ((~0ull) >> (64 - lane));
}

__host__ __device__ inline size_t lds_bytes(int n_lds_nodes, int stack_depth, int stride) {
  return (size_t)n_lds_nodes * sizeof(DNode) + (size_t)stack_depth * stride * 8;
}

#ifndef RT_KSCENE
#define RT_KSCENE 1
#endif
#ifndef RT_NARROW_WAVES
#define RT_NARROW_WAVES 4
#endif
constexpr int kNarrowWaves = RT_NARROW_WAVES;
#ifndef RT_NARROW_WAVES_EXT
#define RT_NARROW_WAVES_EXT 3
#endif

#ifndef RT_HOP_MIN_LANES
#define RT_HOP_MIN_LANES 40
#endif
#ifndef RT_HOP2_INSIDE
#define RT_HOP2_INSIDE 1
#endif
#ifndef RT_HOP2_MIN_LANES_A
#define RT_HOP2_MIN_LANES_A 24
#endif
#ifndef RT_HOP2_MIN_LANES_B
#define RT_HOP2_MIN_LANES_B 16
#endif
#ifndef RT_HOPD_MIN_LANES_A
#define RT_HOPD_MIN_LANES_A 32
#endif
#ifndef RT_HOPD_MIN_LANES_B
#define RT_HOPD_MIN_LANES_B 16
#endif
#ifndef RT_HOPD_MIN_LANES_C
#define RT_HOPD_MIN_LANES_C 16
#endif
#ifndef RT_HOP3_MIN_LANES_A
#define RT_HOP3_MIN_LANES_A RT_HOP2_MIN_LANES_A
#endif
#ifndef RT_HOP3_MIN_LANES_B
#define RT_HOP3_MIN_LANES_B RT_HOP2_MIN_LANES_B
#endif
#ifdef RT_HOP_SERVE_SHARED
struct ServeOut {
  v3 o, d;
  uint32_t draw, c2, c3;
};
__device__ __noinline__ ServeOut hop_serve_ool(const DPrim* lds_prims, const DMat* mats, int prim, int face, v3 o, v3 d,
                                               double t, Rng rng, uint64_t seed_v) {
  DScene S{};
  const uint64_t seed = uniform64(seed_v);
  const DPrim pr = lds_prims[prim];
  Hit hh;
  hit_record<false, false>(S, pr, face, o, d, t, rng, seed, hh);
  const v3 ru = draw_diel(rng, seed);
  const v3 ud = unit_fast(d);
  shade_dielectric(mats[pr.material], ru, ud, rng, o, d, hh);
  return ServeOut{o, d, rng.draw, rng.c2, rng.c3};
}
#endif
template <int THREADS, int MODE, bool EXT, bool LIST = false, int HOP = 0>
__global__ __launch_bounds__(THREADS, THREADS >= kTraceThreadsWide3 ? 1 : (EXT ? RT_NARROW_WAVES_EXT : kNarrowWaves))
void trace_kernel(KParams P) {
  extern __shared__ unsigned char lds_raw[];
  const int tid = threadIdx.x;
  typedef typename Node4Sel<EXT>::T N4;
  N4* lds_nodes = reinterpret_cast<N4*>(lds_raw);
  DPrim* lds_prims = reinterpret_cast<DPrim*>(lds_raw + (size_t)P.scene.n_lds_nodes4 * sizeof(N4));
  const DPerlin* lds_perlin = (MODE == kSceneLds && P.scene.n_lds_perlin > 0)
                                  ? reinterpret_cast<const DPerlin*>(lds_prims + P.scene.n_lds_prims)
                                  : nullptr;
  unsigned char* stk_base = lds_raw + (size_t)P.scene.n_lds_nodes4 * sizeof(N4) +
                            (MODE == kSceneLds ? (size_t)P.scene.n_lds_prims * sizeof(DPrim) +
                                                     (size_t)P.scene.n_lds_perlin * sizeof(DPerlin) +
                                                     (size_t)P.scene.n_lds_mats * sizeof(DMat) +
                                                     (size_t)P.scene.n_lds_texs * sizeof(DTex)
                                               : 0);
  unsigned* stk = reinterpret_cast<unsigned*>(stk_base) + tid;
  stage_nodes4<MODE>(P.scene, lds_nodes, lds_prims);
  const DMat* mats = P.scene.mats;
  const DTex* texs = P.scene.texs;
  if constexpr (MODE == kSceneLds) {
    mats = reinterpret_cast<const DMat*>(reinterpret_cast<const DPerlin*>(lds_prims + P.scene.n_lds_prims) +
                                         P.scene.n_lds_perlin);
    texs = reinterpret_cast<const DTex*>(mats + P.scene.n_lds_mats);
  }

  const DCamera& C = P.cam;
  const DWork& W = P.work;
  const uint64_t seed = W.seed;
  const int lane = __lane_id();

  unsigned long long w_next = 0, w_end = 0;
  bool exhausted = false;
  uint32_t seg;
  {
    const uint32_t per_xcd = (W.n_segs + 7u) / 8u, s0 = (blockIdx.x % 8u) * per_xcd + blockIdx.x / 8u;
    seg = s0 < W.n_segs ? s0 : blockIdx.x % max(W.n_segs, 1u);
  }

  bool has_unit = false, active = false;
  uint32_t pxy = 0;
  int s_end = 0;
  uint32_t part_index = 0;
  v3 sum = V(0, 0, 0), o = V(0, 0, 0), d = V(0, 0, 0), att = V(0, 0, 0), em = V(0, 0, 0);
  int depth_left = 0;
  Rng rng{0, 0, 0, 0, 0};
  unsigned long long n_seg = 0, n_samp = 0;
  unsigned visits = 0, ptests = 0;

#ifdef RT_PHASE_TIMING
  unsigned long long ph_t[kPhBuckets] = {}, ph_last = clock64(), ph_lane_steps = 0, ph_wave_steps = 0;
#define PH_STAMP(b)                               \
  do {                                            \
    const unsigned long long ph_now = clock64();  \
    ph_t[b] += ph_now - ph_last;                  \
    ph_last = ph_now;                             \
  } while (0)
#else
#define PH_STAMP(b) \
  do {              \
  } while (0)
#endif
#ifdef RT_TIMELINE
  const unsigned wave_gid = blockIdx.x * (THREADS / kWave) + tid / kWave;
  bool ph_exh_seen = false;
  if (lane == 0 && wave_gid < (unsigned)kTimelineWaves) g_wave_t0[wave_gid] = __builtin_amdgcn_s_memrealtime();
#endif
  for (;;) {
#if defined(RT_PHASE_TIMING) && !defined(RT_PHASE_NO_EVENTS)
    const unsigned long long ph_before = ph_lane_steps;
#endif
    const DScene& S = P.scene;
    bool hit = false, need_pn = false, need_r = false;
    int prim = -1, face = -1, leaf = -1, mat = 0, ptab = 0, mk = -1;
    double t_best = __builtin_inf(), psc = 0.0;
    Hit h;
    h.point = V(0.0, 0.0, 0.0);
    h.normal = h.point;
    h.t = h.u = h.v = 0.0;
    h.front_face = false;
    PH_COUNT(6);
    n_seg += __popcll(__ballot(active));
    bool waiting = false;
    if constexpr (HOP == 3) {
      static_assert(MODE == kSceneLds && !EXT, "the hop pass is built for the scene-in-LDS reference-scene instances");
      if (active)
        prim = traverse4<THREADS, MODE, EXT>(S, lds_nodes, lds_prims, o, d, 0.001, t_best, face, stk, rng, seed, visits,
                                             ptests RT_STAT_ARG(ph_lane_steps));
      PH_STAMP(kPhTrav);
      GGround* g = (GGround*)kblock(P.kconst)->ground;
      bool pend = false;
      if (active && prim >= 0 && mats[lds_prims[prim].material].kind == RT_MAT_DIELECTRIC)
        for (int i = 0; i < g->n; ++i) pend = pend || g->prim[i] == prim;
#if defined(RT_PHASE_TIMING) && !defined(RT_PHASE_NO_EVENTS)
      if (pend) PH_COUNT(31);
#endif
#pragma unroll 1
      for (int run = 0; run < 3; ++run) {
        if (__popcll(__ballot(pend)) <
            (run == 0 ? RT_HOPD_MIN_LANES_A : (run == 1 ? RT_HOPD_MIN_LANES_B : RT_HOPD_MIN_LANES_C)))
          break;
        int kind = kHopRefused;
        if (pend) {
          PH_COUNT(36 + 4 * run);
          pend = false;
#ifdef RT_HOP_SERVE_SHARED
          const ServeOut so = hop_serve_ool(lds_prims, mats, prim, face, o, d, t_best, rng, seed);
          o = so.o, d = so.d, rng.draw = so.draw, rng.c2 = so.c2, rng.c3 = so.c3;
#else
          const DPrim pr = lds_prims[prim];
          Hit hh;
          hit_record<false, false>(S, pr, face, o, d, t_best, rng, seed, hh);
          const v3 ru = draw_diel(rng, seed);
          const v3 ud = unit_fast(d);
          shade_dielectric(mats[pr.material], ru, ud, rng, o, d, hh);
#endif
          if (--depth_left <= 0) {
            sum = sum + em;
            active = false;
          }
          const bool inward = face < 0 || d.y < 0.0 || box_inward(face, d);
          prim = -1;
          waiting = active;
          if (active && inward) {
            double t_hop;
            int p_hop, f_hop;
            bool guarded;
            kind = ground_hop_t<true>(S, lds_prims, mats, g, o, d, 0.001, t_hop, p_hop, f_hop, guarded);
            if (kind != kHopRefused) {
              prim = p_hop;
              face = f_hop;
              t_best = t_hop;
              waiting = false;
              pend = kind == kHopServed;
              if (pend) PH_COUNT(37 + 4 * run); else PH_COUNT(38 + 4 * run);
            }
          }
          if (waiting) PH_COUNT(39 + 4 * run);
        }
        n_seg += __popcll(__ballot(kind != kHopRefused));
      }
      PH_STAMP(kPhTrav);
    }
    if (active) {
      if constexpr (HOP != 3)
        prim = traverse4<THREADS, MODE, EXT>(S, lds_nodes, lds_prims, o, d, 0.001, t_best, face, stk, rng, seed, visits,
                                        ptests RT_STAT_ARG(ph_lane_steps));
#ifdef RT_PHASE_TIMING
    }
    PH_STAMP(kPhTrav);
    {
#endif
      if (prim >= 0) {
        PH_COUNT(15);
        hit = true;
        const DPrim pr = (MODE == kSceneLds) ? lds_prims[prim] : S.prims[prim];
        hit_record<false, EXT>(S, pr, face, o, d, t_best, rng, seed, h);
        mat = pr.material;
        mk = mats[mat].kind;
        need_r = mk == RT_MAT_LAMBERTIAN || mk == RT_MAT_METAL || mk == RT_MAT_FAIRY_LIGHT || mk == RT_MAT_ISOTROPIC;
        if (mk == RT_MAT_LAMBERTIAN || mk == RT_MAT_FAIRY_LIGHT || mk == RT_MAT_DIFFUSE_LIGHT || mk == RT_MAT_ISOTROPIC) {
          leaf = resolve_texture_t(texs, mats[mat].tex, h.point);
          const DTex& tx = texs[leaf];
          if (tx.kind == RT_TEX_PERLIN) {
            need_pn = true;
            ptab = tx.table;
            psc = tx.scale;
          }
        }
      }
    }
    PH_STAMP(kPhRecord);
#if defined(RT_PHASE_TIMING) && !defined(RT_PHASE_NO_EVENTS)
    if constexpr (HOP == 2) {
      bool dg = false;
      if (hit && mk == RT_MAT_DIELECTRIC) {
        GGround* g = (GGround*)kblock(P.kconst)->ground;
        for (int i = 0; i < g->n; ++i) dg = dg || g->prim[i] == prim;
      }
      const int n_dg = __popcll(__ballot(dg));
      if (dg) {
        PH_COUNT(31);
        if (n_dg >= 8) PH_COUNT(32);
        if (n_dg >= 16) PH_COUNT(33);
        if (n_dg >= 24) PH_COUNT(34);
        if (n_dg >= 32) PH_COUNT(35);
      }
    }
#endif
    const bool ends = active && !waiting && (!hit || mk == RT_MAT_DIFFUSE_LIGHT);
    const bool free_lane = !active || ends;
    bool publish = false;
    uint32_t pub_index = 0;
    if (free_lane && has_unit && rng.sample + 1u >= (uint32_t)s_end) {
      publish = true;
      pub_index = part_index;
      has_unit = false;
    }
    bool need = free_lane && !has_unit;
    unsigned long long mask = __ballot(need);
    if (mask != 0ull && !exhausted) {
      unsigned long long k = __popcll(mask);
      unsigned long long rank = __popcll(mask & lanemask_lt());
      unsigned long long avail = w_end - w_next;
      unsigned long long idx;
      unsigned win = kSegmentWindow;
      if (avail >= k) {
        idx = w_next + rank;
        w_next += k;
      } else {
        KBlk* kb = kblock(P.kconst);
        unsigned long long nb = kb->work.n_units;
        if (kb->work.n_segs != 0u) {
        unsigned* ctr = reinterpret_cast<unsigned*>(kb->unit_counter);
        for (;;) {
          unsigned off = 0;
          if (lane == 0) off = atomicAdd(ctr + seg, kSegmentWindow);
          off = (unsigned)__builtin_amdgcn_readfirstlane((int)off);
          const uint32_t seg_len = kb->work.seg_len;
          const unsigned long long n_units = kb->work.n_units;
          if (off < seg_len && (unsigned long long)seg * seg_len + off < n_units) {
            nb = (unsigned long long)seg * seg_len + off;
            break;
          }
          bool found = false;
          const uint32_t n_segs = kb->work.n_segs;
          for (uint32_t base = 0; base < n_segs; base += kWave) {
            uint32_t cand = seg + 1u + base + (uint32_t)lane;
// ... 77 lines not shown
    PH_STAMP(kPhDraws);
    if (regen) {
      PH_COUNT(11);
      camera_ray_drawn(kblock(P.kconst)->cam, jx, jy, rs, o, d);
    }
    PH_STAMP(kPhCamera);
    if (active && !waiting) {
      bool alive, has_emit = false;
      v3 mul = V(1.0, 1.0, 1.0), emit = V(0.0, 0.0, 0.0);
      if (hit) {
        const DMat& m = mats[mat];
        alive = shade_factor(S, texs, m, leaf, pn, rs, un, rng, o, d, h, prim, face, mul, emit, has_emit);
      } else {
        PH_COUNT(20);
#if RT_KSCENE
        emit = sky_unit(kblock(P.kconst)->scene, un);
#else
        emit = sky_unit(S, un);
#endif
        has_emit = true;
        alive = false;
      }
      if (has_emit) em = em + hmul(att, emit);
      att = hmul(att, mul);
      if (alive) alive = --depth_left > 0;
      if (!alive) {
        sum = sum + em;
        active = false;
      }
    }
    PH_STAMP(kPhShade);
    if (publish) {
      PH_COUNT(24);
      double* dst = kblock(P.kconst)->partial + (size_t)pub_index * 3;
      dst[0] = sum.x;
      dst[1] = sum.y;
      dst[2] = sum.z;
      sum = V(0.0, 0.0, 0.0);
    }
    if (regen) {
      att = V(1.0, 1.0, 1.0);
      em = V(0.0, 0.0, 0.0);
      depth_left = kblock(P.kconst)->work.max_depth;
      active = true;
    }
    PH_STAMP(kPhTail);
    if constexpr (HOP == 1) {
      static_assert(MODE == kSceneLds && !EXT, "the hop pass is built for the scene-in-LDS reference-scene instances");
      bool cand = active && !regen && hit;
      if (cand) cand = lds_prims[prim].kind != kPrimSphere;
      if (__popcll(__ballot(cand)) >= RT_HOP_MIN_LANES) {
        bool serve = false;
        double t_hop = __builtin_inf();
        int p_hop = -1, f_hop = -1;
        if (cand) {
          PH_COUNT(26);
#ifdef RT_HOP_ROOT_OUTLINE
          const RootHit rh = traverse4_root_ool<MODE>(lds_nodes, lds_prims, S.prims, S.root4, S.key_mask, S.origin_limit,
                                                      o, d, rng, seed);
          serve = rh.ok != 0;
          t_hop = rh.t;
          p_hop = rh.best;
          f_hop = rh.face;
#else
          serve = traverse4_root<MODE>(S, lds_nodes, lds_prims, o, d, 0.001, t_hop, p_hop, f_hop, rng, seed, visits, ptests);
#endif
          if (serve) serve = mats[lds_prims[p_hop].material].kind == RT_MAT_DIELECTRIC;
        }
        n_seg += __popcll(__ballot(serve));
        if (serve) {
          PH_COUNT(27);
          const DPrim pr = lds_prims[p_hop];
          Hit hh;
          hit_record<false, false>(S, pr, f_hop, o, d, t_hop, rng, seed, hh);
          const v3 ru = draw_diel(rng, seed);
          const v3 ud = unit_fast(d);
          shade_dielectric(mats[pr.material], ru, ud, rng, o, d, hh);
          if (--depth_left <= 0) {
            sum = sum + em;
            active = false;
          }
        }
      }
      PH_STAMP(kPhTail);
    }
    if constexpr (HOP == 2 || HOP == 3) {
      static_assert(MODE == kSceneLds && !EXT, "the hop pass is built for the scene-in-LDS reference-scene instances");
      bool cand = active && !regen && hit;
      if (cand) cand = lds_prims[prim].kind != kPrimSphere;
#if RT_HOP2_INSIDE
      if (cand && face >= 0) cand = box_inward(face, d);
#endif
#pragma unroll 1
      for (int run = 0; run < 2; ++run) {
        if (__popcll(__ballot(cand)) < (HOP == 3 ? (run ? RT_HOP3_MIN_LANES_B : RT_HOP3_MIN_LANES_A)
                                                 : (run ? RT_HOP2_MIN_LANES_B : RT_HOP2_MIN_LANES_A)))
          break;
        bool serve = false;
        double t_hop = __builtin_inf();
        int p_hop = -1, f_hop = -1;
        if (cand) {
          if (run) PH_COUNT(28); else PH_COUNT(26);
          bool guarded;
          serve = ground_hop(S, lds_prims, mats, (GGround*)kblock(P.kconst)->ground, o, d, 0.001, t_hop, p_hop, f_hop, guarded);
          if (guarded) PH_COUNT(30);
        }
        n_seg += __popcll(__ballot(serve));
        if (serve) {
          if (run) PH_COUNT(29); else PH_COUNT(27);
#ifdef RT_HOP_SERVE_SHARED
          if constexpr (HOP == 3) {
            const ServeOut so = hop_serve_ool(lds_prims, mats, p_hop, f_hop, o, d, t_hop, rng, seed);
            o = so.o, d = so.d, rng.draw = so.draw, rng.c2 = so.c2, rng.c3 = so.c3;
          } else
#endif
          {
          const DPrim pr = lds_prims[p_hop];
          Hit hh;
          hit_record<false, false>(S, pr, f_hop, o, d, t_hop, rng, seed, hh);
          const v3 ru = draw_diel(rng, seed);
          const v3 ud = unit_fast(d);
          shade_dielectric(mats[pr.material], ru, ud, rng, o, d, hh);
          }
          if (--depth_left <= 0) {
            sum = sum + em;
            active = false;
          }
        }
        cand = serve && active;
#if RT_HOP2_INSIDE
        if (cand) cand = box_inward(f_hop, d);
#endif
      }
      PH_STAMP(kPhTail);
    }
#ifdef RT_TIMELINE
    if (exhausted && !ph_exh_seen) {
      ph_exh_seen = true;
      if (lane == 0 && wave_gid < (unsigned)kTimelineWaves) g_wave_tx[wave_gid] = __builtin_amdgcn_s_memrealtime();
    }
#endif
    if (exhausted && !__any(active || has_unit)) break;
#if defined(RT_PHASE_TIMING) && !defined(RT_PHASE_NO_EVENTS)
    {
      unsigned dl = (unsigned)(ph_lane_steps - ph_before);
      if (dl > 0) atomicAdd(&g_visit_hist[min(dl, 63u)], 1ull);
      for (int off = 32; off > 0; off >>= 1) dl = max(dl, (unsigned)__shfl_xor((int)dl, off));
      ph_wave_steps += dl;
      if (lane == 0 && dl > 0) atomicAdd(&g_wave_visit_hist[min(dl, 63u)], 1ull);
    }
#endif
    if (visits > (1u << 30) || ptests > (1u << 30)) {
      DCounters* cs = kblock(P.kconst)->counters + (blockIdx.x % kCounterSlots);
      atomicAdd(&cs->node_visits, (unsigned long long)visits);
      atomicAdd(&cs->prim_tests, (unsigned long long)ptests);
      visits = ptests = 0;
    }
  }
#ifdef RT_TIMELINE
  if (lane == 0 && wave_gid < (unsigned)kTimelineWaves) g_wave_t1[wave_gid] = __builtin_amdgcn_s_memrealtime();
#endif
  unsigned long long n_vis = visits, n_pt = ptests;
  for (int off = 32; off > 0; off >>= 1) {
    n_vis += __shfl_down(n_vis, off);
    n_pt += __shfl_down(n_pt, off);
  }
#ifdef RT_PHASE_TIMING
  for (int off = 32; off > 0; off >>= 1) ph_lane_steps += __shfl_down(ph_lane_steps, off);
  if (lane == 0) atomicAdd(&kblock(P.kconst)->counters[blockIdx.x % kCounterSlots].pad[kPhLaneSteps], ph_lane_steps);
#endif
  if (lane == 0) {
    DCounters* cs = kblock(P.kconst)->counters + (blockIdx.x % kCounterSlots);
    atomicAdd(&cs->segments, n_seg);
    atomicAdd(&cs->samples, n_samp);
    atomicAdd(&cs->node_visits, n_vis);
    atomicAdd(&cs->prim_tests, n_pt);
#ifdef RT_PHASE_TIMING
    for (int b = 0; b < kPhBuckets; ++b)
      if (b != kPhLaneSteps && b != kPhWaveSteps) atomicAdd(&cs->pad[b], ph_t[b]);
    atomicAdd(&cs->pad[kPhWaveSteps], ph_wave_steps);
#endif
  }
}

__global__ __launch_bounds__(256) void reduce_kernel(const double* __restrict__ partial, int n_chunks,
                                                     int n_tiles_rank, int tiles_x, int ty0, int tile_rank,
                                                     int tile_world, int width, int row0, int row1, int packed,
                                                     int accumulate, double* __restrict__ out) {
  long long i = (long long)blockIdx.x * blockDim.x + threadIdx.x;
  long long n_pix = (long long)n_tiles_rank * kTilePixels;
  if (i >= n_pix) return;
  long long lt = i / kTilePixels;
  int lp = (int)(i % kTilePixels);
  long long gt = lt * tile_world + tile_rank;
  int px = (int)(gt % tiles_x) * kTile + lp % kTile;
  int py = (ty0 + (int)(gt / tiles_x)) * kTile + lp / kTile;
  bool inside = px < width && py >= row0 && py < row1;
  double r = 0.0, g = 0.0, b = 0.0;
  const long long o = packed ? i * 3 : ((long long)(py - row0) * width + px) * 3;
  if (accumulate && (packed || inside)) {
    r = out[o + 0];
    g = out[o + 1];
    b = out[o + 2];
  }
  if (inside) {
#pragma unroll 8
    for (int c = 0; c < n_chunks; ++c) {
      const double* p = partial + ((long long)c * n_pix + i) * 3;
      r += p[0];
      g += p[1];
      b += p[2];
    }
  }
  if (packed || inside) {
    out[o + 0] = r;
    out[o + 1] = g;
    out[o + 2] = b;
// ... 247 lines not shown
  const v3 un = unit_fast(!active ? V(1.0, 1.0, 1.0) : (scat && need_r && mk != RT_MAT_METAL) ? rs : d);
  if (!active) return;
  ProbeOut r{};
  r.object = prim;
  bool alive = false, has_emit = false;
  v3 mul = V(1.0, 1.0, 1.0), emit = V(0.0, 0.0, 0.0);
  if (hit) {
    const DMat& m = S.mats[mat];
    alive = shade_factor(S, S.texs, m, leaf, pn, rs, un, rng, o, d, h, prim, face, mul, emit, has_emit);
    r.front_face = h.front_face ? 1 : 0;
    r.t = h.t;
    r.point[0] = h.point.x; r.point[1] = h.point.y; r.point[2] = h.point.z;
    r.normal[0] = h.normal.x; r.normal[1] = h.normal.y; r.normal[2] = h.normal.z;
  } else {
    emit = sky_unit(S, un);
    has_emit = true;
  }
  r.scattered = alive ? 1 : 0;
  r.emits = has_emit ? 1 : 0;
  r.draw = rng.draw;
  r.emitted[0] = emit.x; r.emitted[1] = emit.y; r.emitted[2] = emit.z;
  if (alive) {
    r.attenuation[0] = mul.x; r.attenuation[1] = mul.y; r.attenuation[2] = mul.z;
    r.origin[0] = o.x; r.origin[1] = o.y; r.origin[2] = o.z;
    r.direction[0] = d.x; r.direction[1] = d.y; r.direction[2] = d.z;
  }
  out[i] = r;
}

size_t hit_lds_bytes(int n_lds_nodes, int stack_depth) { return lds_bytes(n_lds_nodes, stack_depth, kHitThreads); }

static int node_mode(const DScene& S) {
  return S.n_lds_nodes >= S.n_nodes ? kNodesLds : (S.n_lds_nodes == 0 ? kNodesGlobal : kNodesMixed);
}

template <int THREADS, int MODE, bool EXT, int HOP = 0>
static hipError_t occupancy_impl1(const DScene& S, int* blocks_per_cu) {
  const size_t lds = trace_lds_bytes(S.n_lds_nodes4, node4_bytes(S.exts != nullptr), S.n_lds_prims, S.n_lds_perlin, S.stack_depth4, THREADS,
                                     S.n_lds_mats, S.n_lds_texs);
  hipError_t e = hipFuncSetAttribute((const void*)trace_kernel<THREADS, MODE, EXT, false, HOP>,
                                     hipFuncAttributeMaxDynamicSharedMemorySize, (int)lds);
  if (e != hipSuccess) return e;
  e = hipFuncSetAttribute((const void*)trace_kernel<THREADS, MODE, EXT, true, HOP>,
                          hipFuncAttributeMaxDynamicSharedMemorySize, (int)lds);
  if (e != hipSuccess) return e;
  return hipOccupancyMaxActiveBlocksPerMultiprocessor(blocks_per_cu, trace_kernel<THREADS, MODE, EXT, false, HOP>, THREADS,
                                                      lds);
}
template <int THREADS, int MODE>
static hipError_t occupancy_impl(const DScene& S, int* blocks_per_cu) {
  return S.exts ? occupancy_impl1<THREADS, MODE, true>(S, blocks_per_cu)
                : occupancy_impl1<THREADS, MODE, false>(S, blocks_per_cu);
}
template <int THREADS, int MODE, bool EXT, int HOP = 0>
static void launch_trace2(const KParams& p, int blocks, size_t lds, hipStream_t stream) {
  if (p.work.tile_list)
    hipLaunchKernelGGL((trace_kernel<THREADS, MODE, EXT, true, HOP>), dim3(blocks), dim3(THREADS), lds, stream, p);
  else
    hipLaunchKernelGGL((trace_kernel<THREADS, MODE, EXT, false, HOP>), dim3(blocks), dim3(THREADS), lds, stream, p);
}
template <int THREADS, int MODE>
static void launch_trace1(const KParams& p, int blocks, size_t lds, hipStream_t stream) {
  if (p.scene.exts)
    launch_trace2<THREADS, MODE, true>(p, blocks, lds, stream);
  else
    launch_trace2<THREADS, MODE, false>(p, blocks, lds, stream);
}

static hipError_t hit_prepare(const DScene& S) {
  const int lds = (int)hit_lds_bytes(S.n_lds_nodes, S.stack_depth);
  switch (node_mode(S)) {
    case kNodesLds: return hipFuncSetAttribute((const void*)hit_kernel<kNodesLds>, hipFuncAttributeMaxDynamicSharedMemorySize, lds);
    case kNodesGlobal: return hipFuncSetAttribute((const void*)hit_kernel<kNodesGlobal>, hipFuncAttributeMaxDynamicSharedMemorySize, lds);
    default: return hipFuncSetAttribute((const void*)hit_kernel<kNodesMixed>, hipFuncAttributeMaxDynamicSharedMemorySize, lds);
  }
}

hipError_t trace_occupancy(const DScene& S, int threads, int hop, int* blocks_per_cu) {
  hipError_t e = hit_prepare(S);
  if (e != hipSuccess) return e;
  if (hop && !(threads == kTraceThreadsWide && !S.exts && S.n_lds_prims > 0)) return hipErrorInvalidValue;
  if (threads == kTraceThreadsWide && !S.exts) {
    if (node_mode4(S) != kNodesLds) return hipErrorInvalidValue;
    if (hop == 3) return occupancy_impl1<kTraceThreadsWide, kSceneLds, false, 3>(S, blocks_per_cu);
    if (hop == 2) return occupancy_impl1<kTraceThreadsWide, kSceneLds, false, 2>(S, blocks_per_cu);
    if (hop) return occupancy_impl1<kTraceThreadsWide, kSceneLds, false, 1>(S, blocks_per_cu);
    if (S.n_lds_prims > 0) return occupancy_impl1<kTraceThreadsWide, kSceneLds, false>(S, blocks_per_cu);
    return occupancy_impl1<kTraceThreadsWide, kNodesLds, false>(S, blocks_per_cu);
  }
  if (threads == kTraceThreadsWide3) {
    if (node_mode4(S) != kNodesLds || !S.exts) return hipErrorInvalidValue;
    if (S.n_lds_prims > 0) return occupancy_impl1<kTraceThreadsWide3, kSceneLds, true>(S, blocks_per_cu);
    return occupancy_impl1<kTraceThreadsWide3, kNodesLds, true>(S, blocks_per_cu);
  }
  switch (node_mode4(S)) {
    case kNodesLds: return occupancy_impl<kTraceThreads, kNodesLds>(S, blocks_per_cu);
    case kNodesGlobal: return occupancy_impl<kTraceThreads, kNodesGlobal>(S, blocks_per_cu);
    default: return occupancy_impl<kTraceThreads, kNodesMixed>(S, blocks_per_cu);
  }
}

hipError_t launch_trace(const KParams& p, int blocks, int threads, int hop, hipStream_t stream) {
  const size_t lds = trace_lds_bytes(p.scene.n_lds_nodes4, node4_bytes(p.scene.exts != nullptr), p.scene.n_lds_prims, p.scene.n_lds_perlin, p.scene.stack_depth4, threads,
                                     p.scene.n_lds_mats, p.scene.n_lds_texs);
  if (hop && !(threads == kTraceThreadsWide && !p.scene.exts && p.scene.n_lds_prims > 0)) return hipErrorInvalidValue;
  if (threads == kTraceThreadsWide && !p.scene.exts) {
    if (hop == 3)
      launch_trace2<kTraceThreadsWide, kSceneLds, false, 3>(p, blocks, lds, stream);
    else if (hop == 2)
      launch_trace2<kTraceThreadsWide, kSceneLds, false, 2>(p, blocks, lds, stream);
    else if (hop)
      launch_trace2<kTraceThreadsWide, kSceneLds, false, 1>(p, blocks, lds, stream);
    else if (p.scene.n_lds_prims > 0)
      launch_trace2<kTraceThreadsWide, kSceneLds, false>(p, blocks, lds, stream);
    else
      launch_trace2<kTraceThreadsWide, kNodesLds, false>(p, blocks, lds, stream);
    return hipGetLastError();
  }
  if (threads == kTraceThreadsWide3) {
    if (!p.scene.exts) return hipErrorInvalidValue;
    if (p.scene.n_lds_prims > 0)
      launch_trace2<kTraceThreadsWide3, kSceneLds, true>(p, blocks, lds, stream);
    else
      launch_trace2<kTraceThreadsWide3, kNodesLds, true>(p, blocks, lds, stream);
    return hipGetLastError();
  }
  switch (node_mode4(p.scene)) {
    case kNodesLds: launch_trace1<kTraceThreads, kNodesLds>(p, blocks, lds, stream); break;
    case kNodesGlobal: launch_trace1<kTraceThreads, kNodesGlobal>(p, blocks, lds, stream); break;
    default: launch_trace1<kTraceThreads, kNodesMixed>(p, blocks, lds, stream);
  }
  return hipGetLastError();
}

hipError_t launch_hit(const DScene& S, const double* rays, int n, double t_min, double t_max, void* out,
                      hipStream_t stream) {
  int blocks = (n + kHitThreads - 1) / kHitThreads;
  if (blocks == 0) return hipSuccess;
  size_t lds = hit_lds_bytes(S.n_lds_nodes, S.stack_depth);
  HitOut* o = static_cast<HitOut*>(out);
  switch (node_mode(S)) {
    case kNodesLds: hipLaunchKernelGGL(hit_kernel<kNodesLds>, dim3(blocks), dim3(kHitThreads), lds, stream, S, rays, n, t_min, t_max, o); break;
    case kNodesGlobal: hipLaunchKernelGGL(hit_kernel<kNodesGlobal>, dim3(blocks), dim3(kHitThreads), lds, stream, S, rays, n, t_min, t_max, o); break;
    default: hipLaunchKernelGGL(hit_kernel<kNodesMixed>, dim3(blocks), dim3(kHitThreads), lds, stream, S, rays, n, t_min, t_max, o);
  }
  return hipGetLastError();
}

hipError_t launch_hit4(const DScene& S, bool wide, const double* rays, int n, double t_min, double t_max, void* out,
                       hipStream_t stream) {
  const int blocks = (n + kHitThreads - 1) / kHitThreads;
  if (blocks == 0) return hipSuccess;
  HitOut* o = static_cast<HitOut*>(out);
  return dispatch_placement<kHitThreads>(S, wide, [&](auto, auto mode) {
    constexpr int M = decltype(mode)::value;
    auto go = [&](auto kernel, bool ext) {
      return launch_block(kernel, blocks, kHitThreads, block_lds_bytes<M>(S, node4_bytes(ext), kHitThreads), stream, S,
                          rays, n, t_min, t_max, o);
    };
    return S.exts ? go(hit4_kernel<M, true>, true) : go(hit4_kernel<M, false>, false);
  });
}

hipError_t launch_probe(const DScene& S, bool wide, const double* rays, int n, uint64_t seed, uint32_t sample,
                        uint32_t draw, void* out, hipStream_t stream) {
  const int blocks = (n + kHitThreads - 1) / kHitThreads;
  if (blocks == 0) return hipSuccess;
  ProbeOut* o = static_cast<ProbeOut*>(out);
  return dispatch_placement<kHitThreads>(S, wide, [&](auto, auto mode) {
    constexpr int M = decltype(mode)::value;
    auto go = [&](auto kernel, bool ext) {
      return launch_block(kernel, blocks, kHitThreads, block_lds_bytes<M>(S, node4_bytes(ext), kHitThreads), stream, S,
                          rays, n, seed, sample, draw, o);
    };
    return S.exts ? go(probe_kernel<M, true>, true) : go(probe_kernel<M, false>, false);
  });
}

hipError_t launch_reduce(const double* partial, int n_chunks, int n_tiles_rank, int tiles_x, int ty0, int tile_rank,
                         int tile_world, int width, int row0, int row1, int packed, int accumulate, double* out,
                         hipStream_t stream) {
  long long n = (long long)n_tiles_rank * kTilePixels;
  int blocks = (int)((n + 255) / 256);
  if (blocks == 0) return hipSuccess;
  hipLaunchKernelGGL(reduce_kernel, dim3(blocks), dim3(256), 0, stream, partial, n_chunks, n_tiles_rank, tiles_x,
                     ty0, tile_rank, tile_world, width, row0, row1, packed, accumulate, out);
  return hipGetLastError();
}

hipError_t launch_fold_stats(const double* partial, int n_chunks, int n_list, const uint32_t* tile_list, int tiles_x,
                             int width, int height, long long n_batches, int batch, double noise_floor,
                             double* accum, double* moments, double* err, hipStream_t stream) {
  const int blocks = (n_list + 3) / 4;
  if (blocks == 0) return hipSuccess;
  hipLaunchKernelGGL(fold_stats_kernel, dim3(blocks), dim3(256), 0, stream, partial, n_chunks, n_list, tile_list,
                     tiles_x, width, height, n_batches, batch, noise_floor, accum, moments, err);
  return hipGetLastError();
}

hipError_t launch_tonemap_counts(const double* accum, const int32_t* counts, int width, int height, uint8_t* rgb8,
                                 hipStream_t stream) {
  const long long n = (long long)width * height * 3;
  const int blocks = (int)((n + 255) / 256);
  if (blocks == 0) return hipSuccess;
  hipLaunchKernelGGL(tonemap_counts_kernel, dim3(blocks), dim3(256), 0, stream, accum, counts, width, height, rgb8);
  return hipGetLastError();
}

hipError_t launch_sum_parts(const double* parts, int n_parts, long long n, double* out, hipStream_t stream) {
  const long long blocks = (n + 255) / 256;
  if (blocks == 0) return hipSuccess;
  hipLaunchKernelGGL(sum_parts_kernel, dim3((unsigned)blocks), dim3(256), 0, stream, parts, n_parts, n, out);
  return hipGetLastError();
}

#ifdef RT_TIMELINE
void timeline_dump() {
  {
    static unsigned long long t0[kTimelineWaves], tx[kTimelineWaves], t1[kTimelineWaves];
    if (hipMemcpyFromSymbol(t0, HIP_SYMBOL(g_wave_t0), sizeof t0) == hipSuccess &&
        hipMemcpyFromSymbol(tx, HIP_SYMBOL(g_wave_tx), sizeof tx) == hipSuccess &&
        hipMemcpyFromSymbol(t1, HIP_SYMBOL(g_wave_t1), sizeof t1) == hipSuccess) {
      std::vector<double> ends, tails, firstx;
      unsigned long long tmin = ~0ull;
      for (int i = 0; i < kTimelineWaves; ++i)
        if (t1[i] && t0[i]) tmin = std::min(tmin, t0[i]);
      for (int i = 0; i < kTimelineWaves; ++i)
        if (t1[i] && t0[i] && t1[i] >= tmin) {
          ends.push_back((double)(t1[i] - tmin) * 1e-2);
          if (tx[i] && tx[i] <= t1[i]) {
            tails.push_back((double)(t1[i] - tx[i]) * 1e-2);
            firstx.push_back((double)(tx[i] - tmin) * 1e-2);
          }
        }
      auto pct = [](std::vector<double> v, double q) {
        if (v.empty()) return 0.0;
        std::sort(v.begin(), v.end());
        return v[std::min(v.size() - 1, (size_t)(q * (double)(v.size() - 1)))];
      };
      fprintf(stderr, "[phase-timeline] waves %zu; exit us p0 %.1f p50 %.1f p90 %.1f p99 %.1f p99.9 %.1f max %.1f; "
              "pool exhausted seen at us p0 %.1f p50 %.1f; exhausted->exit us p50 %.1f p90 %.1f p99 %.1f max %.1f\n",
              ends.size(), pct(ends, 0), pct(ends, 0.5), pct(ends, 0.9), pct(ends, 0.99), pct(ends, 0.999),
              pct(ends, 1), pct(firstx, 0), pct(firstx, 0.5), pct(tails, 0.5), pct(tails, 0.9), pct(tails, 0.99),
              pct(tails, 1));
      std::fill(t0, t0 + kTimelineWaves, 0ull);
      (void)hipMemcpyToSymbol(HIP_SYMBOL(g_wave_t0), t0, sizeof t0);
      (void)hipMemcpyToSymbol(HIP_SYMBOL(g_wave_tx), t0, sizeof t0);
      (void)hipMemcpyToSymbol(HIP_SYMBOL(g_wave_t1), t0, sizeof t0);
    }
  }
}
#endif

#ifdef RT_PHASE_TIMING
void phase_counters_dump() {
  unsigned long long h[2 * kPhaseEvents];
  if (hipMemcpyFromSymbol(h, HIP_SYMBOL(g_phase_ctr), sizeof h) != hipSuccess) return;
  static const char* names[] = {"visit", "visit_with_leaves", "sphere_iter", "sphere_slab_pass", "rect_iter",
                                "pop_iter", "segment_iter", "box_iter", "marble_round", "draws_coop_round",
                                "unit_fetch", "camera_ray", "philox_A", "philox_B", "marble_sin", "hit_record",
                                "checker_level", "dielectric", "metal", "lambertian", "sky", "diffuse_light",
                                "reflectance", "traverse4", "publish", "tie_resolve", "hop_candidate", "hop_served",
                                "hop2_candidate", "hop2_served", "hop_guarded",
                                "down_hit", "down_hit_ge8", "down_hit_ge16", "down_hit_ge24", "down_hit_ge32",
                                "down1_try", "down1_served", "down1_found", "down1_wait",
                                "down2_try", "down2_served", "down2_found", "down2_wait",
                                "down3_try", "down3_served", "down3_found", "down3_wait"};
  static_assert(sizeof names / sizeof names[0] <= kPhaseEvents, "event slots");
  for (int i = 0; i < (int)(sizeof names / sizeof names[0]); ++i)
    if (h[2 * i + 1])
      fprintf(stderr, "[phase-ev] %-18s lanes %.4g waves %.4g lanes/wave %.2f\n", names[i], (double)h[2 * i],
              (double)h[2 * i + 1], (double)h[2 * i] / (double)h[2 * i + 1]);
  unsigned long long lh[64], wh[64];
  if (hipMemcpyFromSymbol(lh, HIP_SYMBOL(g_visit_hist), sizeof lh) == hipSuccess &&
      hipMemcpyFromSymbol(wh, HIP_SYMBOL(g_wave_visit_hist), sizeof wh) == hipSuccess) {
    fprintf(stderr, "[phase-hist] visits: lanes / waves (slowest lane)\n");
    for (int i = 1; i < 64; ++i)
      if (lh[i] || wh[i]) fprintf(stderr, "[phase-hist] %2d %.6g %.6g\n", i, (double)lh[i], (double)wh[i]);
  }
  unsigned long long z[2 * kPhaseEvents] = {};
  (void)hipMemcpyToSymbol(HIP_SYMBOL(g_phase_ctr), z, sizeof z);
  (void)hipMemcpyToSymbol(HIP_SYMBOL(g_visit_hist), z, 64 * sizeof z[0]);
  (void)hipMemcpyToSymbol(HIP_SYMBOL(g_wave_visit_hist), z, 64 * sizeof z[0]);
}
#endif

hipError_t launch_tonemap(const double* accum, int width, int height, double inv, uint8_t* rgb8, hipStream_t stream) {
  const long long n = (long long)width * height * 3;
  const int blocks = (int)((n + 255) / 256);
  if (blocks == 0) return hipSuccess;
  hipLaunchKernelGGL(tonemap_kernel, dim3(blocks), dim3(256), 0, stream, accum, width, height, inv, rgb8);
  return hipGetLastError();
}

hipError_t launch_unpack(const double* gathered, int world, int max_tiles, int n_tiles_total, int tiles_x, int width,
                         int height, double* out, hipStream_t stream) {
  long long n = (long long)world * max_tiles * kTilePixels;
  int blocks = (int)((n + 255) / 256);
  if (blocks == 0) return hipSuccess;
  hipLaunchKernelGGL(unpack_kernel, dim3(blocks), dim3(256), 0, stream, gathered, world, max_tiles, n_tiles_total,
                     tiles_x, width, height, out);
  return hipGetLastError();
}

}
```

### shirley-raytracing-rs_amd/raytracer/_native.py

```python
from __future__ import annotations

import ctypes as C
import os

_PKG_ROOT = os.path.dirname(os.path.dirname(os.path.abspath(__file__)))
LIB_DIR = os.environ.get("SHIRLEY_LIB_DIR") or os.path.join(_PKG_ROOT, "lib")
BIN_DIR = os.path.join(_PKG_ROOT, "bin")

RT_OK, RT_E_INVALID, RT_E_HIP, RT_E_OOM, RT_E_UNSUPPORTED, RT_E_RCCL = 0, 1, 2, 3, 4, 5
RT_COMM_ID_BYTES = 128
RT_GEOM_SPHERE, RT_GEOM_RECT_XY, RT_GEOM_RECT_YZ, RT_GEOM_RECT_XZ, RT_GEOM_RECT_BOX = range(5)
RT_GEOM_MOVING_SPHERE = 5
RT_MAT_METAL, RT_MAT_DIELECTRIC, RT_MAT_LAMBERTIAN, RT_MAT_DIFFUSE_LIGHT, RT_MAT_FAIRY_LIGHT = range(5)
RT_MAT_ISOTROPIC = 5
RT_TEX_SOLID, RT_TEX_CHECKER, RT_TEX_PERLIN, RT_TEX_IMAGE = range(4)
RT_SKY_ABOVE, RT_SKY_FLAT, RT_SKY_NONE = range(3)
RT_BVH_REFERENCE, RT_BVH_SAH = 0, 1
RT_BVH_NODES_GLOBAL, RT_BVH_NODES_HALF_LDS, RT_BVH_NODES_LDS = 0x100, 0x200, 0x400
RT_ENGINE_AUTO, RT_ENGINE_MEGAKERNEL, RT_ENGINE_WAVEFRONT, RT_ENGINE_SPLIT, RT_ENGINE_TIMING = 0, 1, 2, 3, 0x10
RT_TRAVERSAL_BINARY, RT_TRAVERSAL_RENDER = 0, 1
RT_PARTITION_AUTO, RT_PARTITION_TILES, RT_PARTITION_SAMPLES = 0, 1, 2
RT_NEE_MIS = 1

_d3 = C.c_double * 3
# ... 47 lines not shown
                ("sample_begin", C.c_int32), ("sample_count", C.c_int32), ("partition", C.c_int32),
                ("scratch_mb", C.c_int32)]


class rt_scene_stats(C.Structure):
    _fields_ = [("n_objects", C.c_int32), ("n_nodes", C.c_int32), ("n_leaves", C.c_int32),
                ("depth", C.c_int32), ("device_bytes", C.c_int64),
                ("n_nodes4", C.c_int32), ("wide_block", C.c_int32), ("origin_limit", C.c_double),
                ("hop_pass", C.c_int32),
                ("hop_kind", C.c_int32)]


class rt_counters(C.Structure):
    _fields_ = [("samples", C.c_uint64), ("segments", C.c_uint64), ("node_visits", C.c_uint64),
                ("prim_tests", C.c_uint64), ("kernel_ms", C.c_double), ("reduce_ms", C.c_double),
                ("engine", C.c_int32), ("iterations", C.c_int32), ("slots", C.c_uint64),
                ("extend_ms", C.c_double), ("shade_ms", C.c_double), ("texture_ms", C.c_double),
                ("sample_chunk", C.c_int32), ("n_chunks", C.c_int32),
                ("passes", C.c_int32), ("trace_launches", C.c_int32), ("scratch_bytes", C.c_uint64)]


class rt_adaptive_params(C.Structure):
    _fields_ = [("min_samples", C.c_int32), ("step", C.c_int32), ("threshold", C.c_double),
                ("noise_floor", C.c_double)]


class rt_adaptive_report(C.Structure):
    _fields_ = [("steps", C.c_int32), ("tiles", C.c_int32), ("tiles_converged", C.c_int32), ("pad", C.c_int32),
                ("samples", C.c_uint64), ("segments", C.c_uint64), ("kernel_ms", C.c_double),
                ("fold_ms", C.c_double)]


class rt_denoise_inputs(C.Structure):
    _fields_ = [("width", C.c_int32), ("height", C.c_int32), ("samples", C.c_int32), ("feature_samples", C.c_int32),
                ("accum", C.c_void_p), ("counts", C.c_void_p), ("albedo", C.c_void_p), ("normal", C.c_void_p),
                ("depth", C.c_void_p), ("variance", C.c_void_p)]


class rt_denoise_params(C.Structure):
    _fields_ = [("iterations", C.c_int32), ("normal_power_log2", C.c_int32), ("sigma_z", C.c_double),
                ("sigma_a", C.c_double), ("sigma_c", C.c_double), ("albedo_floor", C.c_double)]


class rt_light(C.Structure):
    _fields_ = [("object", C.c_int32), ("geometry", C.c_int32), ("emitter", C.c_int32), ("pad", C.c_int32),
                ("area", C.c_double), ("color", _d3)]


class rt_light_grid(C.Structure):
    _fields_ = [("n", C.c_int32 * 3), ("n_lights", C.c_int32), ("lo", _d3), ("hi", _d3)]


class rt_bvh_node(C.Structure):
    _fields_ = [("box", _d6), ("leaf", C.c_int32), ("lhs", C.c_int32), ("rhs", C.c_int32), ("pad", C.c_int32)]


class rt_hit(C.Structure):
    _fields_ = [("object", C.c_int32), ("front_face", C.c_int32), ("t", C.c_double), ("point", _d3),
                ("normal", _d3), ("u", C.c_double), ("v", C.c_double)]


class rt_probe(C.Structure):
    _fields_ = [("object", C.c_int32), ("front_face", C.c_int32), ("scattered", C.c_int32), ("emits", C.c_int32),
                ("draw", C.c_uint32), ("pad", C.c_int32), ("t", C.c_double), ("point", _d3), ("normal", _d3),
                ("emitted", _d3), ("attenuation", _d3), ("origin", _d3), ("direction", _d3)]


class sh_camera_spec(C.Structure):
    _fields_ = [("width", C.c_int32), ("ratio_num", C.c_int32), ("ratio_den", C.c_int32),
                ("vfov", C.c_double), ("focal_length", C.c_double), ("has_aperture", C.c_int32),
                ("aperture", C.c_double), ("look_from", _d3), ("look_at", _d3), ("up", _d3),
                ("override_focus", C.c_int32), ("focus_length", C.c_double),
                ("time0", C.c_double), ("time1", C.c_double)]


RT_SIGNATURES = {
    "rt_version": (C.c_char_p, []),
    "rt_device_count": (C.c_int, [C.POINTER(C.c_int32)]),
    "rt_create": (C.c_int, [C.c_int32, C.POINTER(C.c_void_p)]),
    "rt_destroy": (C.c_int, [C.c_void_p]),
    "rt_last_error": (C.c_char_p, [C.c_void_p]),
    "rt_scene_upload": (C.c_int, [C.c_void_p, C.POINTER(rt_scene_desc), C.c_int32]),
    "rt_scene_stats_get": (C.c_int, [C.c_void_p, C.POINTER(rt_scene_stats)]),
    "rt_scene_digest": (C.c_int, [C.c_void_p, C.POINTER(C.c_uint64)]),
    "rt_scene_digest_host": (C.c_int, [C.POINTER(rt_scene_desc), C.c_int32, C.POINTER(C.c_uint64)]),
    "rt_render": (C.c_int, [C.c_void_p, C.POINTER(rt_camera), C.POINTER(rt_render_params), C.c_void_p]),
    "rt_render_scanlines": (C.c_int, [C.c_void_p, C.POINTER(rt_camera), C.POINTER(rt_render_params),
                                      C.c_int32, C.c_int32, C.c_void_p]),
    "rt_tile_layout": (C.c_int, [C.POINTER(rt_camera), C.c_int32, C.POINTER(C.c_int32), C.POINTER(C.c_int32)]),
    "rt_render_device": (C.c_int, [C.c_void_p, C.POINTER(rt_camera), C.POINTER(rt_render_params), C.c_void_p,
                                   C.c_void_p]),
    "rt_render_tiles_device": (C.c_int, [C.c_void_p, C.POINTER(rt_camera), C.POINTER(rt_render_params),
                                         C.c_void_p, C.c_void_p]),
    "rt_unpack_tiles_device": (C.c_int, [C.c_void_p, C.POINTER(rt_camera), C.c_int32, C.c_void_p, C.c_void_p,
                                         C.c_void_p]),
    "rt_scene_hit": (C.c_int, [C.c_void_p, C.c_void_p, C.c_int32, C.c_double, C.c_double, C.POINTER(rt_hit)]),
    "rt_scene_hit_ex": (C.c_int, [C.c_void_p, C.c_void_p, C.c_int32, C.c_double, C.c_double, C.c_int32,
                                  C.POINTER(rt_hit)]),
    "rt_probe_segment": (C.c_int, [C.c_void_p, C.c_void_p, C.c_int32, C.c_uint64, C.c_uint32, C.c_uint32,
                                   C.POINTER(rt_probe)]),
    "rt_synchronize": (C.c_int, [C.c_void_p]),
    "rt_comm_unique_id": (C.c_int, [C.c_void_p]),
    "rt_comm_init_rank": (C.c_int, [C.c_void_p, C.c_void_p, C.c_int32, C.c_int32, C.POINTER(C.c_void_p)]),
    "rt_comm_destroy": (C.c_int, [C.c_void_p]),
    "rt_render_sharded": (C.c_int, [C.c_void_p, C.c_void_p, C.POINTER(rt_camera), C.POINTER(rt_render_params),
                                    C.c_void_p, C.c_void_p]),
    "rt_render_multi": (C.c_int, [C.POINTER(C.c_void_p), C.c_int32, C.POINTER(rt_camera), C.POINTER(rt_render_params),
                                  C.c_void_p]),
    "rt_counters_get": (C.c_int, [C.c_void_p, C.POINTER(rt_counters)]),
    "rt_bvh_build_host": (C.c_int, [C.POINTER(rt_scene_desc), C.c_int32, C.POINTER(C.c_int32),
                                    C.POINTER(rt_bvh_node), C.POINTER(C.c_int32)]),
    "rt_tonemap": (C.c_int, [C.c_void_p, C.c_int32, C.c_int32, C.c_int32, C.c_void_p]),
    "rt_tonemap_device": (C.c_int, [C.c_void_p, C.c_void_p, C.c_int32, C.c_int32, C.c_int32, C.c_void_p,
                                    C.c_void_p]),
    "rt_render_adaptive": (C.c_int, [C.c_void_p, C.POINTER(rt_camera), C.POINTER(rt_render_params),
                                     C.POINTER(rt_adaptive_params), C.c_void_p, C.c_void_p, C.c_void_p, C.c_void_p,
                                     C.POINTER(rt_adaptive_report)]),
    "rt_tonemap_counts": (C.c_int, [C.c_void_p, C.c_void_p, C.c_int32, C.c_int32, C.c_void_p]),
    "rt_tonemap_counts_device": (C.c_int, [C.c_void_p, C.c_void_p, C.c_void_p, C.c_int32, C.c_int32, C.c_void_p,
                                           C.c_void_p]),
    "rt_render_features": (C.c_int, [C.c_void_p, C.POINTER(rt_camera), C.POINTER(rt_render_params), C.c_int32,
                                     C.c_void_p, C.c_void_p, C.c_void_p]),
    "rt_render_features_device": (C.c_int, [C.c_void_p, C.POINTER(rt_camera), C.POINTER(rt_render_params), C.c_int32,
                                            C.c_void_p, C.c_void_p, C.c_void_p, C.c_void_p]),
    "rt_denoise": (C.c_int, [C.POINTER(rt_denoise_inputs), C.POINTER(rt_denoise_params), C.c_void_p]),
    "rt_denoise_device": (C.c_int, [C.c_void_p, C.POINTER(rt_denoise_inputs), C.POINTER(rt_denoise_params),
                                    C.c_void_p, C.c_void_p]),
    "rt_moments_variance": (C.c_int, [C.c_void_p, C.c_void_p, C.c_int32, C.c_int32, C.c_int32, C.c_void_p]),
    "rt_moments_variance_device": (C.c_int, [C.c_void_p, C.c_void_p, C.c_void_p, C.c_int32, C.c_int32, C.c_int32,
                                             C.c_void_p, C.c_void_p]),
    "rt_scene_occluded": (C.c_int, [C.c_void_p, C.c_void_p, C.c_int32, C.c_double, C.c_double, C.c_void_p,
                                    C.c_void_p]),
    "rt_scene_occluded_device": (C.c_int, [C.c_void_p, C.c_void_p, C.c_int32, C.c_double, C.c_double, C.c_void_p,
                                           C.c_void_p, C.c_void_p]),
    "rt_render_ao": (C.c_int, [C.c_void_p, C.POINTER(rt_camera), C.POINTER(rt_render_params), C.c_int32, C.c_double,
                               C.c_void_p]),
    "rt_render_ao_device": (C.c_int, [C.c_void_p, C.POINTER(rt_camera), C.POINTER(rt_render_params), C.c_int32,
                                      C.c_double, C.c_void_p, C.c_void_p]),
    "rt_scene_lights": (C.c_int, [C.c_void_p, C.POINTER(C.c_int32), C.POINTER(C.c_int32), C.POINTER(rt_light)]),
    "rt_scene_lights_host": (C.c_int, [C.POINTER(rt_scene_desc), C.POINTER(C.c_int32), C.POINTER(C.c_int32),
                                       C.POINTER(rt_light)]),
    "rt_render_direct": (C.c_int, [C.c_void_p, C.POINTER(rt_camera), C.POINTER(rt_render_params), C.c_int32,
                                   C.c_void_p, C.c_void_p]),
    "rt_render_direct_device": (C.c_int, [C.c_void_p, C.POINTER(rt_camera), C.POINTER(rt_render_params), C.c_int32,
                                          C.c_void_p, C.c_void_p, C.c_void_p]),
    "rt_render_nee": (C.c_int, [C.c_void_p, C.POINTER(rt_camera), C.POINTER(rt_render_params), C.c_int32,
                                C.c_void_p]),
    "rt_render_nee_device": (C.c_int, [C.c_void_p, C.POINTER(rt_camera), C.POINTER(rt_render_params), C.c_int32,
                                       C.c_void_p, C.c_void_p]),
    "rt_light_grid_host": (C.c_int, [C.POINTER(rt_scene_desc), C.c_int32, C.POINTER(rt_light_grid), C.c_void_p]),
    "rt_scene_light_pick": (C.c_int, [C.c_void_p, C.c_int32, C.POINTER(rt_light_grid)]),
    "rt_light_pick_at": (C.c_int, [C.c_void_p, C.c_int32, C.c_void_p, C.c_void_p, C.c_void_p, C.c_void_p]),
}

SH_SIGNATURES = {
    "sh_last_error": (C.c_char_p, []),
    "sh_scene_new": (C.c_void_p, []),
    "sh_scene_free": (None, [C.c_void_p]),
    "sh_scene_set_skybox": (C.c_int, [C.c_void_p, C.c_int32, C.POINTER(C.c_double)]),
    "sh_scene_add_json": (C.c_int, [C.c_void_p, C.c_char_p]),
    "sh_scene_len": (C.c_int32, [C.c_void_p]),
    "sh_scene_to_json": (C.c_int, [C.c_void_p, C.c_int32, C.c_char_p, C.c_size_t, C.POINTER(C.c_size_t)]),
    "sh_scene_from_json": (C.c_int, [C.c_char_p, C.POINTER(C.c_void_p)]),
    "sh_scene_builtin": (C.c_int, [C.c_char_p, C.c_uint64, C.POINTER(C.c_void_p)]),
    "sh_scene_finalize": (C.c_int, [C.c_void_p, C.c_uint64, C.POINTER(C.c_void_p)]),
    "sh_desc_view": (C.POINTER(rt_scene_desc), [C.c_void_p]),
# ... 62 lines not shown
```

### shirley-raytracing-rs_amd/raytracer/render.py

```python
from __future__ import annotations

import ctypes as C
from dataclasses import dataclass
from typing import Optional

import numpy as np

from . import _native as N
from .scene import Scene


def _check(ctx, code):
    if code != 0:
        raise N.RtError(code, N.rt_lib().rt_last_error(ctx).decode())


@dataclass
class RenderSettings:
    samples: int = 100
    max_reflect: int = 50
    seed: int = 0x5EED
    sample_chunk: int = 0
    tile_rank: int = 0
    tile_world: int = 1
# ... 48 lines not shown
        p.albedo_floor = float(self.albedo_floor)
        return p


def _denoise_inputs(width, height, accum_ptr, albedo_ptr, normal_ptr, depth_ptr, samples, feature_samples,
                    counts_ptr=0, variance_ptr=0) -> N.rt_denoise_inputs:
    i = N.rt_denoise_inputs()
    i.width, i.height, i.samples, i.feature_samples = int(width), int(height), int(samples), int(feature_samples)
    i.accum, i.albedo, i.normal, i.depth = accum_ptr or None, albedo_ptr or None, normal_ptr or None, depth_ptr or None
    i.counts, i.variance = counts_ptr or None, variance_ptr or None
    return i


def denoise(accum: np.ndarray, albedo: np.ndarray, normal: np.ndarray, depth: np.ndarray, samples: int = 0,
            feature_samples: int = 0, settings: Optional[DenoiseSettings] = None,
            counts: Optional[np.ndarray] = None, variance: Optional[np.ndarray] = None) -> np.ndarray:
    h, w, _ = accum.shape
    f64 = lambda a, shape: np.ascontiguousarray(a, dtype=np.float64).reshape(shape)
    a, al, no, de = f64(accum, (h, w, 3)), f64(albedo, (h, w, 3)), f64(normal, (h, w, 3)), f64(depth, (h, w))
    cn = None if counts is None else np.ascontiguousarray(counts, dtype=np.int32).reshape(h, w)
    va = None if variance is None else f64(variance, (h, w))
    out = np.zeros((h, w, 3), dtype=np.float64)
    i = _denoise_inputs(w, h, a.ctypes.data, al.ctypes.data, no.ctypes.data, de.ctypes.data, samples,
                        feature_samples or samples, 0 if cn is None else cn.ctypes.data,
                        0 if va is None else va.ctypes.data)
    p = (settings or DenoiseSettings()).params()
    code = N.rt_lib().rt_denoise(C.byref(i), C.byref(p), out.ctypes.data)
    if code:
        raise N.RtError(code, "rt_denoise: invalid argument")
    return out


def moments_variance(moments: np.ndarray, counts: np.ndarray, batch: int) -> np.ndarray:
    h, w = counts.shape
    m = np.ascontiguousarray(moments, dtype=np.float64).reshape(h, w, 2)
    n = np.ascontiguousarray(counts, dtype=np.int32)
    out = np.zeros((h, w), dtype=np.float64)
    code = N.rt_lib().rt_moments_variance(m.ctypes.data, n.ctypes.data, int(batch) or 4, w, h, out.ctypes.data)
    if code:
        raise N.RtError(code, "rt_moments_variance: invalid argument")
    return out


class Device:

    def __init__(self, device: int = 0):
        lib = N.rt_lib()
        h = C.c_void_p()
        code = lib.rt_create(int(device), C.byref(h))
        if code != 0:
            raise N.RtError(code, f"rt_create(device={device}) failed: no usable HIP device")
        self._h = h
        self.scene: Optional[Scene] = None

    def close(self):
        if getattr(self, "_h", None):
            N.rt_lib().rt_destroy(self._h)
            self._h = None

    __del__ = close

    @property
    def handle(self):
        return self._h

    def upload(self, scene: Scene, bvh: str = "reference", nodes: str = "auto") -> "Device":
        builder = {"reference": N.RT_BVH_REFERENCE, "sah": N.RT_BVH_SAH}[bvh]
        builder |= {"auto": 0, "global": N.RT_BVH_NODES_GLOBAL, "half-lds": N.RT_BVH_NODES_HALF_LDS,
                    "lds": N.RT_BVH_NODES_LDS}[nodes]
        _check(self._h, N.rt_lib().rt_scene_upload(self._h, scene.desc_ptr, builder))
        self.scene = scene
        return self

    def digest(self) -> int:
        d = C.c_uint64()
        _check(self._h, N.rt_lib().rt_scene_digest(self._h, C.byref(d)))
        return d.value

    def stats(self) -> N.rt_scene_stats:
        s = N.rt_scene_stats()
        _check(self._h, N.rt_lib().rt_scene_stats_get(self._h, C.byref(s)))
        return s

    def render(self, camera: N.rt_camera, settings: RenderSettings) -> np.ndarray:
        out = np.zeros((camera.image_height, camera.image_width, 3), dtype=np.float64)
        p = settings.params()
        _check(self._h, N.rt_lib().rt_render(self._h, C.byref(camera), C.byref(p), out.ctypes.data))
        return out

    def render_adaptive(self, camera: N.rt_camera, settings: RenderSettings, adaptive: AdaptiveSettings):
        h, w = camera.image_height, camera.image_width
        accum = np.zeros((h, w, 3), dtype=np.float64)
        counts = np.zeros((h, w), dtype=np.int32)
        moments = np.zeros((h, w, 2), dtype=np.float64)
        tile_error = np.zeros(((h + 7) // 8, (w + 7) // 8), dtype=np.float64)
        report = N.rt_adaptive_report()
        p, a = settings.params(), adaptive.params()
        _check(self._h, N.rt_lib().rt_render_adaptive(self._h, C.byref(camera), C.byref(p), C.byref(a),
                                                      accum.ctypes.data, counts.ctypes.data, moments.ctypes.data,
                                                      tile_error.ctypes.data, C.byref(report)))
        return accum, counts, moments, tile_error, report

    def render_features(self, camera: N.rt_camera, settings: RenderSettings, chain: int = 8):
        h, w = camera.image_height, camera.image_width
        albedo = np.zeros((h, w, 3), dtype=np.float64)
        normal = np.zeros((h, w, 3), dtype=np.float64)
        depth = np.zeros((h, w), dtype=np.float64)
        p = settings.params()
        _check(self._h, N.rt_lib().rt_render_features(self._h, C.byref(camera), C.byref(p), int(chain),
                                                      albedo.ctypes.data, normal.ctypes.data, depth.ctypes.data))
        return albedo, normal, depth

    def render_features_device(self, camera, settings: RenderSettings, chain: int, albedo_ptr: int, normal_ptr: int,
                               depth_ptr: int, stream: int = 0):
        p = settings.params()
        _check(self._h, N.rt_lib().rt_render_features_device(
            self._h, C.byref(camera), C.byref(p), int(chain), C.c_void_p(albedo_ptr or None),
            C.c_void_p(normal_ptr or None), C.c_void_p(depth_ptr or None), C.c_void_p(stream or None)))

    def denoise_device(self, width: int, height: int, accum_ptr: int, albedo_ptr: int, normal_ptr: int,
                       depth_ptr: int, out_ptr: int, samples: int = 0, feature_samples: int = 0,
                       settings: Optional[DenoiseSettings] = None, counts_ptr: int = 0, variance_ptr: int = 0,
                       stream: int = 0):
        i = _denoise_inputs(width, height, accum_ptr, albedo_ptr, normal_ptr, depth_ptr, samples,
                            feature_samples or samples, counts_ptr, variance_ptr)
        p = (settings or DenoiseSettings()).params()
        _check(self._h, N.rt_lib().rt_denoise_device(self._h, C.byref(i), C.byref(p), C.c_void_p(out_ptr or None),
                                                     C.c_void_p(stream or None)))

    def moments_variance_device(self, moments_ptr: int, counts_ptr: int, batch: int, width: int, height: int,
                                out_ptr: int, stream: int = 0):
        _check(self._h, N.rt_lib().rt_moments_variance_device(
            self._h, C.c_void_p(moments_ptr or None), C.c_void_p(counts_ptr or None), int(batch) or 4, int(width),
            int(height), C.c_void_p(out_ptr or None), C.c_void_p(stream or None)))

    def tonemap_counts_device(self, accum_ptr: int, counts_ptr: int, width: int, height: int, rgb8_ptr: int,
                              stream: int = 0):
        _check(self._h, N.rt_lib().rt_tonemap_counts_device(self._h, C.c_void_p(accum_ptr), C.c_void_p(counts_ptr),
                                                            int(width), int(height), C.c_void_p(rgb8_ptr),
                                                            C.c_void_p(stream or None)))

    def render_scanlines(self, camera: N.rt_camera, settings: RenderSettings, line_begin: int,
                         line_end: int) -> np.ndarray:
        out = np.zeros((max(0, line_end - line_begin), camera.image_width, 3), dtype=np.float64)
        p = settings.params()
        _check(self._h, N.rt_lib().rt_render_scanlines(self._h, C.byref(camera), C.byref(p), line_begin, line_end,
                                                       out.ctypes.data))
        return out

    def render_device(self, camera, settings: RenderSettings, accum_ptr: int, stream: int = 0):
        p = settings.params()
        _check(self._h, N.rt_lib().rt_render_device(self._h, C.byref(camera), C.byref(p), C.c_void_p(accum_ptr),
                                                    C.c_void_p(stream or None)))

    def render_tiles_device(self, camera, settings: RenderSettings, packed_ptr: int, stream: int = 0):
        p = settings.params()
        _check(self._h, N.rt_lib().rt_render_tiles_device(self._h, C.byref(camera), C.byref(p),
                                                          C.c_void_p(packed_ptr), C.c_void_p(stream or None)))

    def unpack_tiles_device(self, camera, world: int, gathered_ptr: int, accum_ptr: int, stream: int = 0):
        _check(self._h, N.rt_lib().rt_unpack_tiles_device(self._h, C.byref(camera), int(world),
                                                          C.c_void_p(gathered_ptr), C.c_void_p(accum_ptr),
                                                          C.c_void_p(stream or None)))

    def tonemap_device(self, accum_ptr: int, width: int, height: int, samples: int, rgb8_ptr: int,
                       stream: int = 0):
# ... 225 lines not shown
```

Before: 3136.

## Add sorted-plane hop instance for stacked ground boxes in the trace kernel

Adds a compiled plane table (sorted y-levels with packed prim/face/answer info) for stacked ground box scenes, plus a new HOP==4 kernel instance. That instance answers the down pass and the hop pass with a linear scan over planes instead of the general ground_hop routine. It is enabled when the hop-down conditions hold and the plane gaps are valid, and it also adds phase-timing counters. The goal is to cut per-ray cost of the hop tests. The risks are a new template instance with different register and occupancy behaviour, and possible mismatches with the general path.

```diff
diff --git a/include/shirley_rt.h b/include/shirley_rt.h
--- a/include/shirley_rt.h
+++ b/include/shirley_rt.h
@@ -173,6 +173,7 @@
 
 int rt_scene_upload(rt_ctx* ctx, const rt_scene_desc* scene, int32_t bvh_builder);
 int rt_scene_stats_get(rt_ctx* ctx, rt_scene_stats* out);
+int rt_scene_hop_instance(rt_ctx* ctx, int32_t* out);
 int rt_scene_digest(rt_ctx* ctx, uint64_t* out);
 int rt_scene_digest_host(const rt_scene_desc* scene, int32_t bvh_builder, uint64_t* out);
 
diff --git a/shirley-raytracing-rs_amd/csrc/rt/rt_api.cpp b/shirley-raytracing-rs_amd/csrc/rt/rt_api.cpp
--- a/shirley-raytracing-rs_amd/csrc/rt/rt_api.cpp
+++ b/shirley-raytracing-rs_amd/csrc/rt/rt_api.cpp
@@ -394,6 +394,7 @@
     kb.unit_counter = kp.unit_counter;
     kb.counters = kp.counters;
     kb.ground = c->place.hop_kind == 2 ? static_cast<const DGround*>(c->ground.p) : nullptr;
+    kb.planes = c->place.hop_planes ? static_cast<const DPlanes*>(c->planes.p) : nullptr;
     void* kdev = static_cast<KBlock*>(c->kcam.p) + k;
     HIP_TRY(c, hipMemcpyAsync(kdev, &kb, sizeof(KBlock), hipMemcpyHostToDevice, s));
     kp.kconst = (uint64_t)(uintptr_t)kdev;
@@ -473,7 +474,7 @@
   if (!c) return RT_OK;
   (void)hipSetDevice(c->device);
   if (c->stream) (void)hipStreamSynchronize(c->stream);
-  for (DevBuf* b : {&c->nodes, &c->nodes4, &c->prims, &c->mats, &c->texs, &c->perlin, &c->texels, &c->exts, &c->ground, &c->lights, &c->prim_light, &c->light_cdf, &c->partial, &c->kcam, &c->shutter0, &c->moments, &c->tile_list, &c->tile_err, &c->dn_a, &c->dn_b, &c->feat,
+  for (DevBuf* b : {&c->nodes, &c->nodes4, &c->prims, &c->mats, &c->texs, &c->perlin, &c->texels, &c->exts, &c->ground, &c->planes, &c->lights, &c->prim_light, &c->light_cdf, &c->partial, &c->kcam, &c->shutter0, &c->moments, &c->tile_list, &c->tile_err, &c->dn_a, &c->dn_b, &c->feat,
                     &c->accum, &c->counters, &c->unit_counter, &c->wf_pool, &c->wf_iters, &c->packed, &c->gathered,
                     &c->parts, &c->band, &c->digests})
     release(*b);
@@ -515,6 +516,11 @@
     if ((st = up(c->ground, cs.ground))) return st;
   } else {
     release(c->ground);
+  }
+  if (!cs.planes.empty()) {
+    if ((st = up(c->planes, cs.planes))) return st;
+  } else {
+    release(c->planes);
   }
   if (!cs.lights.dev.empty()) {
     if ((st = up(c->lights, cs.lights.dev))) return st;
@@ -608,6 +614,13 @@
   return RT_OK;
 }
 
+int rt_scene_hop_instance(rt_ctx* c, int32_t* out) {
+  if (!c || !out) return RT_E_INVALID;
+  if (!c->have_scene) return fail(c, RT_E_INVALID, "no scene uploaded");
+  *out = hop_instance(c->place);
+  return RT_OK;
+}
+
 int rt_tile_layout(const rt_camera* cam, int32_t world, int32_t* n_tiles_total, int32_t* max_tiles_per_rank) {
   if (!cam || world < 1 || cam->image_width < 1 || cam->image_height < 1) return RT_E_INVALID;
   int tiles_y = (cam->image_height + kTile - 1) / kTile;
@@ -774,12 +787,12 @@
     double ph[kPhBuckets] = {};
     for (const DCounters& k : dc)
       for (int i = 0; i < kPhBuckets; ++i) ph[i] += (double)k.pad[i];
-    const int order[] = {kPhTrav, kPhRecord, kPhRegen, kPhMarble, kPhDraws, kPhCamera, kPhShade, kPhTail};
-    const char* names[] = {"trav", "record", "regen", "marble", "draws", "camera", "shade", "tail"};
+    const int order[] = {kPhTrav, kPhDown, kPhRecord, kPhRegen, kPhMarble, kPhDraws, kPhCamera, kPhShade, kPhTail, kPhHop};
+    const char* names[] = {"trav", "down", "record", "regen", "marble", "draws", "camera", "shade", "tail", "hop"};
     double tot = 0;
     for (int b : order) tot += ph[b];
     fprintf(stderr, "[phase] wave-time fractions:");
-    for (int i = 0; i < 8; ++i) fprintf(stderr, " %s %.4f", names[i], ph[order[i]] / tot);
+    for (int i = 0; i < 10; ++i) fprintf(stderr, " %s %.4f", names[i], ph[order[i]] / tot);
     fprintf(stderr, " (wave-cycles %.4g)\n", tot);
     const double lane = ph[kPhLaneSteps], wave = ph[kPhWaveSteps];
     fprintf(stderr, "[phase] traversal lane steps %.4g, wave steps %.4g, SIMD utilisation %.3f\n", lane, wave,
diff --git a/shirley-raytracing-rs_amd/csrc/rt/rt_ctx.h b/shirley-raytracing-rs_amd/csrc/rt/rt_ctx.h
--- a/shirley-raytracing-rs_amd/csrc/rt/rt_ctx.h
+++ b/shirley-raytracing-rs_amd/csrc/rt/rt_ctx.h
@@ -40,6 +40,7 @@
   rt::DScene scene{};
   DevBuf nodes, nodes4, prims, mats, texs, perlin, texels, exts;
   DevBuf ground;
+  DevBuf planes;
   DevBuf lights;
   DevBuf prim_light;
   std::vector<rt_light> light_list;
diff --git a/shirley-raytracing-rs_amd/csrc/rt/rt_device.h b/shirley-raytracing-rs_amd/csrc/rt/rt_device.h
--- a/shirley-raytracing-rs_amd/csrc/rt/rt_device.h
+++ b/shirley-raytracing-rs_amd/csrc/rt/rt_device.h
@@ -858,9 +858,11 @@
 
 #ifdef RT_PHASE_TIMING
 #define g_trav_lane_steps trav_lane_steps_ref
-constexpr int kPhaseEvents = 48;
+constexpr int kPhaseEvents = 52;
 static __device__ unsigned long long g_phase_ctr[2 * kPhaseEvents];
 static __device__ unsigned long long g_visit_hist[64], g_wave_visit_hist[64];
+enum : int { kHopClkDownServe = 0, kHopClkDownNext = 1, kHopClkHopNext = 2, kHopClkHopServe = 3, kHopClks = 4 };
+static __device__ unsigned long long g_hop_clk[kHopClks];
 
 __device__ __forceinline__ void ph_count(int i) {
   const unsigned long long act = __ballot(1);
@@ -1378,6 +1380,51 @@
 __device__ __forceinline__ bool ground_hop(const DScene& S, const DPrim* lds_prims, const DMat* mats, GGround* g, v3 o, v3 d,
                                            double t_min, double& t_best, int& best, int& face_best, bool& guarded) {
   return ground_hop_t<false>(S, lds_prims, mats, g, o, d, t_min, t_best, best, face_best, guarded) != kHopRefused;
+}
+
+typedef __attribute__((address_space(4))) const DPlanes GPlanes;
+template <bool DOWN>
+__device__ __forceinline__ int plane_hop_t(GGround* g, GPlanes* pl, v3 o, v3 d, double t_min, double& t_best, int& best,
+                                           int& face_best, bool& guarded) {
+  guarded = false;
+  const double ay = fabs(d.y);
+  const double x0 = pl->x0, x1 = pl->x1, z0 = pl->z0, z1 = pl->z1;
+  const bool slab_ok = o.y >= g->y_lo && o.y <= g->y_hi && ay >= g->dy_min && ay <= 0x1p300 &&
+                       d.x * d.x + d.z * d.z <= g->ratio2 * (d.y * d.y);
+  if (!(slab_ok && o.x >= x0 && o.x <= x1 && o.z >= z0 && o.z <= z1)) return kHopRefused;
+  const bool up = d.y > 0.0;
+  const double tol = pl->tol, hi = o.y + tol, lo = o.y - tol;
+  double y = 0.0;
+  int info = -1;
+  const int n = pl->n;
+#pragma unroll 1
+  for (int k = 0; k < n; ++k) {
+    const double yk = pl->y[k];
+    const bool take = up ? (yk > hi && info < 0) : yk < lo;
+    y = take ? yk : y;
+    info = take ? pl->info[k] : info;
+  }
+  const int kind = info < 0 ? kHopRefused : ((info >> 2) & 3);
+  if (kind == kHopRefused || (!DOWN && kind != kHopServed)) return kHopRefused;
+  const double t = div_recip(y - o.y, Recip{d.y, div_recip(1.0, recip(d.y))});
+  if (!(t > 2.0 * t_min)) return kHopRefused;
+  const double hx = o.x + t * d.x, hz = o.z + t * d.z;
+  if (!(hx >= x0 && hx <= x1 && hz >= z0 && hz <= z1)) return kHopRefused;
+  if ((info & 16) && kind == kHopServed) {
+    const int nx = g->nx;
+    const int ix = ground_cell(hx, g->x0, nx), iz = ground_cell(hz, g->z0, g->nz);
+    if (ix >= 0 && iz >= 0) {
+      typedef __attribute__((address_space(1))) const uint32_t GBits;
+      const unsigned c = (unsigned)iz * (unsigned)nx + (unsigned)ix;
+      GBits* bits = (GBits*)(uintptr_t)((uint64_t)(uintptr_t)g + sizeof(DGround));
+      guarded = (bits[c >> 5] >> (c & 31u)) & 1u;
+      if (guarded) return kHopRefused;
+    }
+  }
+  t_best = t;
+  best = (int)((unsigned)info >> 5);
+  face_best = (info & 3) == 0 ? -1 : 3 + (info & 3);
+  return kind;
 }
 
 struct Trav4 {
diff --git a/shirley-raytracing-rs_amd/csrc/rt/rt_layout.h b/shirley-raytracing-rs_amd/csrc/rt/rt_layout.h
--- a/shirley-raytracing-rs_amd/csrc/rt/rt_layout.h
+++ b/shirley-raytracing-rs_amd/csrc/rt/rt_layout.h
@@ -173,6 +173,16 @@
   return (q >= 0.0 && q < (double)n) ? (int)q : -1;
 }
 
+constexpr int kGroundMaxPlanes = 2 * kGroundMaxPrims;
+struct alignas(16) DPlanes {
+  double x0, x1, z0, z1;
+  double tol;
+  int32_t n, pad;
+  double y[kGroundMaxPlanes];
+  int32_t info[kGroundMaxPlanes];
+};
+static_assert(sizeof(DPlanes) == 144, "DPlanes layout");
+
 struct DCamera {
   int32_t width, height;
   int32_t has_lens;
@@ -219,8 +229,12 @@
 constexpr int kCounterSlots = 64;
 enum : int {
   kPhRegen = 0, kPhTrav = 1, kPhShade = 2, kPhLaneSteps = 3, kPhWaveSteps = 4, kPhRecord = 5, kPhMarble = 6,
-  kPhDraws = 7, kPhCamera = 8, kPhTail = 9, kPhBuckets = 10
-};
+  kPhDraws = 7, kPhCamera = 8, kPhTail = 9,
+  kPhDown = 10,
+  kPhHop = 11,
+  kPhBuckets = 12
+};
+static_assert(kPhBuckets <= (int)(sizeof(DCounters::pad) / sizeof(unsigned long long)), "DCounters.pad slots");
 
 struct KParams {
   DScene scene;
@@ -241,6 +255,7 @@
   unsigned long long* unit_counter;
   DCounters* counters;
   const DGround* ground;
+  const DPlanes* planes;
 };
 
 struct WfState {
diff --git a/shirley-raytracing-rs_amd/csrc/rt/scene_compile.cpp b/shirley-raytracing-rs_amd/csrc/rt/scene_compile.cpp
--- a/shirley-raytracing-rs_amd/csrc/rt/scene_compile.cpp
+++ b/shirley-raytracing-rs_amd/csrc/rt/scene_compile.cpp
@@ -37,6 +37,7 @@
   if (const char* e = getenv("SHIRLEY_HOP")) {
     t.hop_root = std::strcmp(e, "root") == 0;
     t.hop_up = std::strcmp(e, "up") == 0;
+    t.hop_general = std::strcmp(e, "general") == 0;
   }
   if (const char* e = getenv("SHIRLEY_SAH_BOXW")) t.sah_box_weight = atof(e);
   t.sah_binned = getenv("SHIRLEY_SAH_BINNED") != nullptr;
@@ -516,7 +517,10 @@
 namespace {
 
 bool sphere_never_hit(const double* p) { return p[3] <= 0.0 && p[1] - p[3] >= p[1] + p[3]; }
-bool ground_stack(const std::vector<DPrim>& prims, int n_prims, std::vector<uint32_t>& out) {
+struct GroundConsts {
+  double gap = 0.0, tol = 0.0, reach = 0.0, ext = 0.0;
+};
+bool ground_stack(const std::vector<DPrim>& prims, int n_prims, std::vector<uint32_t>& out, GroundConsts* consts = nullptr) {
   out.clear();
   std::vector<int32_t> boxes, rects;
   double top = -std::numeric_limits<double>::infinity(), low = -top;
@@ -576,6 +580,12 @@
   const double gap = 4.0 * eta + 4.0 * tol;
   for (double y : planes)
     if (y != top && !(y <= top - gap)) return false;
+  if (consts) {
+    consts->gap = gap;
+    consts->tol = tol;
+    consts->reach = reach;
+    consts->ext = std::max(std::max(std::fabs(ex0), std::fabs(ex1)), std::max(std::fabs(ez0), std::fabs(ez1)));
+  }
 
   DGround g;
   std::memset(&g, 0, sizeof g);
@@ -623,6 +633,56 @@
         }
       }
   }
+  return true;
+}
+
+bool plane_stack(const std::vector<DPrim>& prims, const std::vector<DMat>& mats, const std::vector<uint32_t>& ground,
+                 const GroundConsts& k, std::vector<uint32_t>& out) {
+  out.clear();
+  DGround g;
+  std::memcpy(&g, ground.data(), sizeof g);
+  const double inf = std::numeric_limits<double>::infinity();
+  double x0 = -inf, x1 = inf, z0 = -inf, z1 = inf;
+  struct Plane {
+    double y;
+    int32_t info;
+  };
+  std::vector<Plane> pl;
+  auto info = [](int32_t prim, int face, int answer, bool top) {
+    return (int32_t)((uint32_t)prim << 5 | (top ? 16u : 0u) | (uint32_t)answer << 2 | (face < 0 ? 0u : (face == 4 ? 1u : 2u)));
+  };
+  for (int i = 0; i < g.n; ++i) {
+    const int32_t leaf = g.prim[i];
+    if (leaf < 0 || leaf >= (1 << 26)) return false;
+    const DPrim& q = prims[leaf];
+    const double* p = q.p;
+    const bool diel = mats[q.material].kind == RT_MAT_DIELECTRIC;
+    if (i < g.n_box) {
+      x0 = std::max(x0, p[0]), x1 = std::min(x1, p[3]), z0 = std::max(z0, p[2]), z1 = std::min(z1, p[5]);
+      for (int face = 4; face <= 5; ++face) {
+        const double y = face == 4 ? p[4] : p[1];
+        pl.push_back({y, info(leaf, face, diel ? 1 : (y <= g.y_down ? 2 : 0), y == g.y_top)});
+      }
+    } else {
+      x0 = std::max(x0, p[0]), x1 = std::min(x1, p[1]), z0 = std::max(z0, p[2]), z1 = std::min(z1, p[3]);
+      pl.push_back({p[4], info(leaf, -1, (!diel && p[4] + 0.0001 <= g.y_down) ? 2 : 0, false)});
+    }
+  }
+  std::stable_sort(pl.begin(), pl.end(), [](const Plane& a, const Plane& b) { return a.y < b.y; });
+  for (size_t i = 1; i < pl.size(); ++i)
+    if (!(pl[i].y - pl[i - 1].y > k.gap)) return false;
+  const double mx = 0x1p-44 * (k.ext + k.reach + 1.0);
+  DPlanes d;
+  std::memset(&d, 0, sizeof d);
+  d.x0 = x0 + mx, d.x1 = x1 - mx, d.z0 = z0 + mx, d.z1 = z1 - mx;
+  if (!(d.x0 < d.x1 && d.z0 < d.z1)) return false;
+  if (g.nx > 0 && !(g.x0 >= d.x0 && g.x0 + g.nx * kGroundCell <= d.x1 && g.z0 >= d.z0 && g.z0 + g.nz * kGroundCell <= d.z1))
+    return false;
+  d.tol = k.tol;
+  d.n = (int32_t)pl.size();
+  for (size_t i = 0; i < pl.size(); ++i) d.y[i] = pl[i].y, d.info[i] = pl[i].info;
+  out.assign(sizeof(DPlanes) / 4, 0u);
+  std::memcpy(out.data(), &d, sizeof d);
   return true;
 }
 
@@ -680,7 +740,8 @@
     coat = o.geometry == RT_GEOM_RECT_BOX && d->materials[o.material].kind == RT_MAT_DIELECTRIC;
   }
   P.hop_pass = coat && !ext && prims_lds && !tune.no_hop;
-  P.hop_kind = !P.hop_pass ? 0 : (!tune.hop_root && ground_stack(cs.prims, d->n_objects, cs.ground)) ? 2 : 1;
+  GroundConsts consts;
+  P.hop_kind = !P.hop_pass ? 0 : (!tune.hop_root && ground_stack(cs.prims, d->n_objects, cs.ground, &consts)) ? 2 : 1;
   if (P.hop_kind != 2) cs.ground.clear();
   P.hop_down = false;
   if (P.hop_kind == 2 && !tune.hop_up) {
@@ -692,6 +753,8 @@
       P.hop_down = i < g.n_box ? (q.p[1] <= g.y_down || q.p[4] <= g.y_down) : q.p[4] + 0.0001 <= g.y_down;
     }
   }
+  P.hop_planes = P.hop_down && !tune.hop_general && plane_stack(cs.prims, cs.mats, cs.ground, consts, cs.planes);
+  if (!P.hop_planes) cs.planes.clear();
 
   const long long wf_stack = (long long)wf_extend_lds(0, P.stack_depth);
   if (wf_stack > kLdsBytes)
diff --git a/shirley-raytracing-rs_amd/csrc/rt/scene_compile.h b/shirley-raytracing-rs_amd/csrc/rt/scene_compile.h
--- a/shirley-raytracing-rs_amd/csrc/rt/scene_compile.h
+++ b/shirley-raytracing-rs_amd/csrc/rt/scene_compile.h
@@ -25,6 +25,7 @@
   bool no_hop = false;
   bool hop_root = false;
   bool hop_up = false;
+  bool hop_general = false;
   double sah_box_weight = 4.0;
   bool sah_binned = false;
   bool wf_extend2 = false;
@@ -49,9 +50,12 @@
   bool hop_pass = false;
   int hop_kind = 0;
   bool hop_down = false;
+  bool hop_planes = false;
 };
 
-inline int hop_instance(const ScenePlacement& P) { return P.hop_kind == 2 && P.hop_down ? 3 : P.hop_kind; }
+inline int hop_instance(const ScenePlacement& P) {
+  return P.hop_kind == 2 && P.hop_down ? (P.hop_planes ? 4 : 3) : P.hop_kind;
+}
 
 inline void place_scene(const ScenePlacement& P, DScene& S) {
   S.stack_depth = P.stack_depth;
@@ -95,6 +99,7 @@
   std::vector<uint8_t> texels;
   std::vector<size_t> img_off;
   std::vector<uint32_t> ground;
+  std::vector<uint32_t> planes;
   std::vector<int32_t> prim_object;
   std::vector<std::pair<int32_t, std::pair<double, double>>> uv_fixups;
   LightList lights;
diff --git a/shirley-raytracing-rs_amd/csrc/rt/trace.hip b/shirley-raytracing-rs_amd/csrc/rt/trace.hip
--- a/shirley-raytracing-rs_amd/csrc/rt/trace.hip
+++ b/shirley-raytracing-rs_amd/csrc/rt/trace.hip
@@ -54,6 +54,21 @@
 #endif
 #ifndef RT_HOP3_MIN_LANES_B
 #define RT_HOP3_MIN_LANES_B RT_HOP2_MIN_LANES_B
+#endif
+#ifndef RT_HOP4D_MIN_LANES_A
+#define RT_HOP4D_MIN_LANES_A 24
+#endif
+#ifndef RT_HOP4D_MIN_LANES_B
+#define RT_HOP4D_MIN_LANES_B RT_HOPD_MIN_LANES_B
+#endif
+#ifndef RT_HOP4D_MIN_LANES_C
+#define RT_HOP4D_MIN_LANES_C RT_HOPD_MIN_LANES_C
+#endif
+#ifndef RT_HOP4_MIN_LANES_A
+#define RT_HOP4_MIN_LANES_A 16
+#endif
+#ifndef RT_HOP4_MIN_LANES_B
+#define RT_HOP4_MIN_LANES_B 8
 #endif
 #ifdef RT_HOP_SERVE_SHARED
 struct ServeOut {
@@ -131,9 +146,23 @@
     ph_t[b] += ph_now - ph_last;                  \
     ph_last = ph_now;                             \
   } while (0)
+  unsigned long long ph_part_last = 0;
+#define PH_PART_BEGIN() ph_part_last = clock64()
+#define PH_PART(b)                                                                                                \
+  do {                                                                                                            \
+    const unsigned long long ph_now = clock64();                                                                  \
+    if ((int)__lane_id() == __builtin_ctzll(__ballot(1))) atomicAdd(&g_hop_clk[b], ph_now - ph_part_last);        \
+    ph_part_last = ph_now;                                                                                        \
+  } while (0)
 #else
 #define PH_STAMP(b) \
   do {              \
+  } while (0)
+#define PH_PART_BEGIN() \
+  do {                  \
+  } while (0)
+#define PH_PART(b) \
+  do {             \
   } while (0)
 #endif
 #ifdef RT_TIMELINE
@@ -157,7 +186,7 @@
     PH_COUNT(6);
     n_seg += __popcll(__ballot(active));
     bool waiting = false;
-    if constexpr (HOP == 3) {
+    if constexpr (HOP >= 3) {
       static_assert(MODE == kSceneLds && !EXT, "the hop pass is built for the scene-in-LDS reference-scene instances");
       if (active)
         prim = traverse4<THREADS, MODE, EXT>(S, lds_nodes, lds_prims, o, d, 0.001, t_best, face, stk, rng, seed, visits,
@@ -173,11 +202,13 @@
 #pragma unroll 1
       for (int run = 0; run < 3; ++run) {
         if (__popcll(__ballot(pend)) <
-            (run == 0 ? RT_HOPD_MIN_LANES_A : (run == 1 ? RT_HOPD_MIN_LANES_B : RT_HOPD_MIN_LANES_C)))
+            (HOP == 4 ? (run == 0 ? RT_HOP4D_MIN_LANES_A : (run == 1 ? RT_HOP4D_MIN_LANES_B : RT_HOP4D_MIN_LANES_C))
+                      : (run == 0 ? RT_HOPD_MIN_LANES_A : (run == 1 ? RT_HOPD_MIN_LANES_B : RT_HOPD_MIN_LANES_C))))
           break;
         int kind = kHopRefused;
         if (pend) {
           PH_COUNT(36 + 4 * run);
+          PH_PART_BEGIN();
           pend = false;
 #ifdef RT_HOP_SERVE_SHARED
           const ServeOut so = hop_serve_ool(lds_prims, mats, prim, face, o, d, t_best, rng, seed);
@@ -195,13 +226,18 @@
             active = false;
           }
           const bool inward = face < 0 || d.y < 0.0 || box_inward(face, d);
+          PH_PART(kHopClkDownServe);
           prim = -1;
           waiting = active;
           if (active && inward) {
+            PH_COUNT(48 + run);
             double t_hop;
             int p_hop, f_hop;
             bool guarded;
-            kind = ground_hop_t<true>(S, lds_prims, mats, g, o, d, 0.001, t_hop, p_hop, f_hop, guarded);
+            if constexpr (HOP == 4)
+              kind = plane_hop_t<true>(g, (GPlanes*)kblock(P.kconst)->planes, o, d, 0.001, t_hop, p_hop, f_hop, guarded);
+            else
+              kind = ground_hop_t<true>(S, lds_prims, mats, g, o, d, 0.001, t_hop, p_hop, f_hop, guarded);
             if (kind != kHopRefused) {
               prim = p_hop;
               face = f_hop;
@@ -211,14 +247,15 @@
               if (pend) PH_COUNT(37 + 4 * run); else PH_COUNT(38 + 4 * run);
             }
           }
+          PH_PART(kHopClkDownNext);
           if (waiting) PH_COUNT(39 + 4 * run);
         }
         n_seg += __popcll(__ballot(kind != kHopRefused));
       }
-      PH_STAMP(kPhTrav);
+      PH_STAMP(kPhDown);
     }
     if (active) {
-      if constexpr (HOP != 3)
+      if constexpr (HOP < 3)
         prim = traverse4<THREADS, MODE, EXT>(S, lds_nodes, lds_prims, o, d, 0.001, t_best, face, stk, rng, seed, visits,
                                         ptests RT_STAT_ARG(ph_lane_steps));
 #ifdef RT_PHASE_TIMING
@@ -462,9 +499,9 @@
           }
         }
       }
-      PH_STAMP(kPhTail);
-    }
-    if constexpr (HOP == 2 || HOP == 3) {
+      PH_STAMP(kPhHop);
+    }
+    if constexpr (HOP >= 2) {
       static_assert(MODE == kSceneLds && !EXT, "the hop pass is built for the scene-in-LDS reference-scene instances");
       bool cand = active && !regen && hit;
       if (cand) cand = lds_prims[prim].kind != kPrimSphere;
@@ -473,21 +510,29 @@
 #endif
 #pragma unroll 1
       for (int run = 0; run < 2; ++run) {
-        if (__popcll(__ballot(cand)) < (HOP == 3 ? (run ? RT_HOP3_MIN_LANES_B : RT_HOP3_MIN_LANES_A)
-                                                 : (run ? RT_HOP2_MIN_LANES_B : RT_HOP2_MIN_LANES_A)))
+        if (__popcll(__ballot(cand)) < (HOP == 4   ? (run ? RT_HOP4_MIN_LANES_B : RT_HOP4_MIN_LANES_A)
+                                        : HOP == 3 ? (run ? RT_HOP3_MIN_LANES_B : RT_HOP3_MIN_LANES_A)
+                                                   : (run ? RT_HOP2_MIN_LANES_B : RT_HOP2_MIN_LANES_A)))
           break;
         bool serve = false;
         double t_hop = __builtin_inf();
         int p_hop = -1, f_hop = -1;
         if (cand) {
           if (run) PH_COUNT(28); else PH_COUNT(26);
+          PH_PART_BEGIN();
           bool guarded;
-          serve = ground_hop(S, lds_prims, mats, (GGround*)kblock(P.kconst)->ground, o, d, 0.001, t_hop, p_hop, f_hop, guarded);
+          if constexpr (HOP == 4)
+            serve = plane_hop_t<false>((GGround*)kblock(P.kconst)->ground, (GPlanes*)kblock(P.kconst)->planes, o, d, 0.001, t_hop,
+                                       p_hop, f_hop, guarded) != kHopRefused;
+          else
+            serve = ground_hop(S, lds_prims, mats, (GGround*)kblock(P.kconst)->ground, o, d, 0.001, t_hop, p_hop, f_hop, guarded);
+          PH_PART(kHopClkHopNext);
           if (guarded) PH_COUNT(30);
         }
         n_seg += __popcll(__ballot(serve));
         if (serve) {
           if (run) PH_COUNT(29); else PH_COUNT(27);
+          PH_PART_BEGIN();
 #ifdef RT_HOP_SERVE_SHARED
           if constexpr (HOP == 3) {
             const ServeOut so = hop_serve_ool(lds_prims, mats, p_hop, f_hop, o, d, t_hop, rng, seed);
@@ -506,13 +551,14 @@
             sum = sum + em;
             active = false;
           }
+          PH_PART(kHopClkHopServe);
         }
         cand = serve && active;
 #if RT_HOP2_INSIDE
         if (cand) cand = box_inward(f_hop, d);
 #endif
       }
-      PH_STAMP(kPhTail);
+      PH_STAMP(kPhHop);
     }
 #ifdef RT_TIMELINE
     if (exhausted && !ph_exh_seen) {
@@ -926,6 +972,7 @@
   if (hop && !(threads == kTraceThreadsWide && !S.exts && S.n_lds_prims > 0)) return hipErrorInvalidValue;
   if (threads == kTraceThreadsWide && !S.exts) {
     if (node_mode4(S) != kNodesLds) return hipErrorInvalidValue;
+    if (hop == 4) return occupancy_impl1<kTraceThreadsWide, kSceneLds, false, 4>(S, blocks_per_cu);
     if (hop == 3) return occupancy_impl1<kTraceThreadsWide, kSceneLds, false, 3>(S, blocks_per_cu);
     if (hop == 2) return occupancy_impl1<kTraceThreadsWide, kSceneLds, false, 2>(S, blocks_per_cu);
     if (hop) return occupancy_impl1<kTraceThreadsWide, kSceneLds, false, 1>(S, blocks_per_cu);
@@ -949,7 +996,9 @@
                                      p.scene.n_lds_mats, p.scene.n_lds_texs);
   if (hop && !(threads == kTraceThreadsWide && !p.scene.exts && p.scene.n_lds_prims > 0)) return hipErrorInvalidValue;
   if (threads == kTraceThreadsWide && !p.scene.exts) {
-    if (hop == 3)
+    if (hop == 4)
+      launch_trace2<kTraceThreadsWide, kSceneLds, false, 4>(p, blocks, lds, stream);
+    else if (hop == 3)
       launch_trace2<kTraceThreadsWide, kSceneLds, false, 3>(p, blocks, lds, stream);
     else if (hop == 2)
       launch_trace2<kTraceThreadsWide, kSceneLds, false, 2>(p, blocks, lds, stream);
@@ -1109,7 +1158,8 @@
                                 "down_hit", "down_hit_ge8", "down_hit_ge16", "down_hit_ge24", "down_hit_ge32",
                                 "down1_try", "down1_served", "down1_found", "down1_wait",
                                 "down2_try", "down2_served", "down2_found", "down2_wait",
-                                "down3_try", "down3_served", "down3_found", "down3_wait"};
+                                "down3_try", "down3_served", "down3_found", "down3_wait",
+                                "down1_ask", "down2_ask", "down3_ask"};
   static_assert(sizeof names / sizeof names[0] <= kPhaseEvents, "event slots");
   for (int i = 0; i < (int)(sizeof names / sizeof names[0]); ++i)
     if (h[2 * i + 1])
@@ -1122,6 +1172,20 @@
     for (int i = 1; i < 64; ++i)
       if (lh[i] || wh[i]) fprintf(stderr, "[phase-hist] %2d %.6g %.6g\n", i, (double)lh[i], (double)wh[i]);
   }
+  unsigned long long hc[kHopClks];
+  if (hipMemcpyFromSymbol(hc, HIP_SYMBOL(g_hop_clk), sizeof hc) == hipSuccess) {
+    const double down_runs = (double)(h[2 * 36 + 1] + h[2 * 40 + 1] + h[2 * 44 + 1]);
+    const double hop_runs = (double)(h[2 * 26 + 1] + h[2 * 28 + 1]), hop_serves = (double)(h[2 * 27 + 1] + h[2 * 29 + 1]);
+    fprintf(stderr, "[phase-run] down pass: runs %.4g, wave-cycles per run: serve body %.1f, next hit (+ guard) %.1f\n", down_runs,
+            down_runs ? (double)hc[kHopClkDownServe] / down_runs : 0.0, down_runs ? (double)hc[kHopClkDownNext] / down_runs : 0.0);
+    fprintf(stderr, "[phase-run] hop pass: runs %.4g, wave-cycles per run: next hit (+ guard) %.1f; serving runs %.4g, serve body %.1f\n",
+            hop_runs, hop_runs ? (double)hc[kHopClkHopNext] / hop_runs : 0.0, hop_serves,
+            hop_serves ? (double)hc[kHopClkHopServe] / hop_serves : 0.0);
+    fprintf(stderr, "[phase-run] wave-cycles in all: down serve %.4g, down next %.4g, hop next %.4g, hop serve %.4g\n", (double)hc[0],
+            (double)hc[1], (double)hc[2], (double)hc[3]);
+    unsigned long long zc[kHopClks] = {};
+    (void)hipMemcpyToSymbol(HIP_SYMBOL(g_hop_clk), zc, sizeof zc);
+  }
   unsigned long long z[2 * kPhaseEvents] = {};
   (void)hipMemcpyToSymbol(HIP_SYMBOL(g_phase_ctr), z, sizeof z);
   (void)hipMemcpyToSymbol(HIP_SYMBOL(g_visit_hist), z, 64 * sizeof z[0]);
diff --git a/shirley-raytracing-rs_amd/raytracer/_native.py b/shirley-raytracing-rs_amd/raytracer/_native.py
--- a/shirley-raytracing-rs_amd/raytracer/_native.py
+++ b/shirley-raytracing-rs_amd/raytracer/_native.py
@@ -153,6 +153,7 @@
     "rt_last_error": (C.c_char_p, [C.c_void_p]),
     "rt_scene_upload": (C.c_int, [C.c_void_p, C.POINTER(rt_scene_desc), C.c_int32]),
     "rt_scene_stats_get": (C.c_int, [C.c_void_p, C.POINTER(rt_scene_stats)]),
+    "rt_scene_hop_instance": (C.c_int, [C.c_void_p, C.POINTER(C.c_int32)]),
     "rt_scene_digest": (C.c_int, [C.c_void_p, C.POINTER(C.c_uint64)]),
     "rt_scene_digest_host": (C.c_int, [C.POINTER(rt_scene_desc), C.c_int32, C.POINTER(C.c_uint64)]),
     "rt_render": (C.c_int, [C.c_void_p, C.POINTER(rt_camera), C.POINTER(rt_render_params), C.c_void_p]),
diff --git a/shirley-raytracing-rs_amd/raytracer/render.py b/shirley-raytracing-rs_amd/raytracer/render.py
--- a/shirley-raytracing-rs_amd/raytracer/render.py
+++ b/shirley-raytracing-rs_amd/raytracer/render.py
@@ -154,6 +154,11 @@
         _check(self._h, N.rt_lib().rt_scene_stats_get(self._h, C.byref(s)))
         return s
 
+    def hop_instance(self) -> int:
+        k = C.c_int32()
+        _check(self._h, N.rt_lib().rt_scene_hop_instance(self._h, C.byref(k)))
+        return k.value
+
     def render(self, camera: N.rt_camera, settings: RenderSettings) -> np.ndarray:
         out = np.zeros((camera.image_height, camera.image_width, 3), dtype=np.float64)
         p = settings.params()
```

New measurement: 3371 (median of 6 runs). 7.5% higher.
